# aicell-lab/bioengine-worker

Measured on AMD Instinct MI355X. Metric: cellpose_cyto3_512x512_imgs_per_sec, higher is better.
Workload: dtype bf16; 1 GPU; model=cellpose-cyto3 CPnet (nbase 2-32-64-128-256, style on, BN folded), global_batch=32, parallelism=dp1 (replica per GPU)

## Files before the change

bioengine_worker_amd/models/cpnet.py:

```python
from __future__ import annotations

import os
from dataclasses import dataclass

import torch
import torch.nn as nn
import torch.nn.functional as F

from ..ops import conv as convops
from ..ops import conv_pair as pairops
from ..ops import style as styleops


def _norm(c: int, kind: str) -> nn.Module:
    if kind == "batch":
        return nn.BatchNorm2d(c, eps=1e-5, momentum=0.05)
    if kind == "group":
        g = 8 if c % 8 == 0 else 1
        return nn.GroupNorm(g, c, eps=1e-5)
    raise ValueError(kind)


def batchconv(cin, cout, sz, norm="batch"):
    return nn.Sequential(_norm(cin, norm), nn.ReLU(inplace=True), nn.Conv2d(cin, cout, sz, padding=sz // 2))


def batchconv0(cin, cout, sz, norm="batch"):
    return nn.Sequential(_norm(cin, norm), nn.Conv2d(cin, cout, sz, padding=sz // 2))


class resdown(nn.Module):
    def __init__(self, cin, cout, sz, norm="batch"):
        super().__init__()
        self.conv = nn.Sequential()
        self.proj = batchconv0(cin, cout, 1, norm)
        for t in range(4):
            self.conv.add_module(f"conv_{t}", batchconv(cin if t == 0 else cout, cout, sz, norm))

    def forward(self, x):
        x = self.proj(x) + self.conv[1](self.conv[0](x))
        x = x + self.conv[3](self.conv[2](x))
        return x


class downsample(nn.Module):
    def __init__(self, nbase, sz, norm="batch"):
        super().__init__()
        self.down = nn.Sequential()
        self.maxpool = nn.MaxPool2d(2, 2)
        for n in range(len(nbase) - 1):
            self.down.add_module(f"res_down_{n}", resdown(nbase[n], nbase[n + 1], sz, norm))

    def forward(self, x):
        xd = []
        for n in range(len(self.down)):
            y = self.maxpool(xd[n - 1]) if n > 0 else x
            xd.append(self.down[n](y))
        return xd


class batchconvstyle(nn.Module):
    def __init__(self, cin, cout, style_channels, sz, norm="batch"):
        super().__init__()
        self.concatenation = False
        self.conv = batchconv(cin, cout, sz, norm)
        self.full = nn.Linear(style_channels, cout)

    def forward(self, style, x, y=None):
        if y is not None:
            x = x + y
        feat = self.full(style)
        return self.conv(x + feat.unsqueeze(-1).unsqueeze(-1))


class resup(nn.Module):
    def __init__(self, cin, cout, style_channels, sz, norm="batch"):
        super().__init__()
        self.conv = nn.Sequential()
        self.conv.add_module("conv_0", batchconv(cin, cout, sz, norm))
        self.conv.add_module("conv_1", batchconvstyle(cout, cout, style_channels, sz, norm))
        self.conv.add_module("conv_2", batchconvstyle(cout, cout, style_channels, sz, norm))
        self.conv.add_module("conv_3", batchconvstyle(cout, cout, style_channels, sz, norm))
        self.proj = batchconv0(cin, cout, 1, norm)

    def forward(self, x, y, style):
        x = self.proj(x) + self.conv[1](style, self.conv[0](x), y=y)
        x = x + self.conv[3](style, self.conv[2](style, x))
        return x


class make_style(nn.Module):
    def __init__(self):
        super().__init__()
        self.flatten = nn.Flatten()

    def forward(self, x0):
        style = F.avg_pool2d(x0, kernel_size=x0.shape[2:])
        style = self.flatten(style)
        return style / torch.sum(style ** 2, dim=1, keepdim=True) ** 0.5


class upsample(nn.Module):
    def __init__(self, nbase, sz, norm="batch"):
        super().__init__()
        self.upsampling = nn.Upsample(scale_factor=2, mode="nearest")
        self.up = nn.Sequential()
        for n in range(1, len(nbase)):
            self.up.add_module(f"res_up_{n - 1}", resup(nbase[n], nbase[n - 1], nbase[-1], sz, norm))

    def forward(self, style, xd):
        x = self.up[-1](xd[-1], xd[-1], style)
        for n in range(len(self.up) - 2, -1, -1):
            x = self.upsampling(x)
            x = self.up[n](x, xd[n], style)
        return x


class CPnet(nn.Module):

    def __init__(self, nbase=(2, 32, 64, 128, 256), nout=3, sz=3, diam_mean=30.0, norm="batch", style_on=True):
        super().__init__()
        nbase = list(nbase)
        self.nbase = nbase
        self.nout = nout
        self.sz = sz
        self.norm_kind = norm
        self.style_on = style_on
        self.downsample = downsample(nbase, sz, norm)
        nbaseup = nbase[1:] + [nbase[-1]]
        self.upsample = upsample(nbaseup, sz, norm)
        self.make_style = make_style()
        self.output = batchconv(nbaseup[0], nout, 1, norm)
        self.diam_mean = nn.Parameter(torch.ones(1) * diam_mean, requires_grad=False)
        self.diam_labels = nn.Parameter(torch.ones(1) * diam_mean, requires_grad=False)

    @property
    def nchan(self):
        return self.nbase[0]

    def forward(self, data):
        T0 = self.downsample(data)
        style = self.make_style(T0[-1])
        style0 = style
        if not self.style_on:
            style = style * 0
        T1 = self.upsample(style, T0)
        T1 = self.output(T1)
        return T1, style0, T0

    def randomize_(self, seed: int = 0) -> "CPnet":
        g = torch.Generator().manual_seed(seed)
        for m in self.modules():
            if isinstance(m, nn.Conv2d):
                fan_in = m.in_channels * m.kernel_size[0] * m.kernel_size[1]
                m.weight.data = torch.randn(m.weight.shape, generator=g) * (1.0 / fan_in) ** 0.5
                if m.bias is not None:
                    m.bias.data = torch.randn(m.bias.shape, generator=g) * 0.01
            elif isinstance(m, nn.Linear):
                m.weight.data = torch.randn(m.weight.shape, generator=g) * (1.0 / m.in_features) ** 0.5
                m.bias.data = torch.randn(m.bias.shape, generator=g) * 0.01
            elif isinstance(m, nn.BatchNorm2d):
                m.weight.data = 1.0 + 0.1 * torch.randn(m.weight.shape, generator=g)
                m.bias.data = 0.1 * torch.randn(m.bias.shape, generator=g)
                m.running_mean.data = 0.1 * torch.randn(m.running_mean.shape, generator=g)
                m.running_var.data = 1.0 + 0.1 * torch.rand(m.running_var.shape, generator=g)
            elif isinstance(m, nn.GroupNorm):
                m.weight.data = 1.0 + 0.1 * torch.randn(m.weight.shape, generator=g)
                m.bias.data = 0.1 * torch.randn(m.bias.shape, generator=g)
        return self



def _bn_fold(bn: nn.Module, device) -> tuple[torch.Tensor, torch.Tensor]:
    if isinstance(bn, nn.BatchNorm2d):
        s = bn.weight.detach().float() / torch.sqrt(bn.running_var.detach().float() + bn.eps)
        t = bn.bias.detach().float() - bn.running_mean.detach().float() * s
        return s.to(device).contiguous(), t.to(device).contiguous()
    raise TypeError("CPnetEngine folds eval-mode BatchNorm only; GroupNorm nets run the autograd path")


def _pad_vec(v: torch.Tensor, n: int, fill: float) -> torch.Tensor:
    if v.numel() == n:
        return v
    out = torch.full((n,), fill, dtype=v.dtype, device=v.device)
    out[: v.numel()] = v
    return out


class _FConv:

    def __init__(self, seq: nn.Sequential, relu: bool, device, cin_pad=None, cout_pad_to=None):
        bn, conv = seq[0], seq[-1]
        self.pc = convops.PackedConv.from_weight(conv.weight, conv.bias, cin_pad=cin_pad, cout_pad_to=cout_pad_to).to(device)
        if convops.pp128_build(self.pc) is not None and torch.device(device).type == "cuda":
            self.pc.frag()
        s, t = _bn_fold(bn, device)
        self.scale = _pad_vec(s, self.pc.cin_pad, 0.0)
        self.shift = _pad_vec(t, self.pc.cin_pad, 0.0)
        self.relu = relu

    def __call__(self, x, *, x2=None, shift=None, residual=None, inmode="none", out_nchw_f32=False, cout_valid=None,
                 residual_mode="full"):
        return convops.fused_conv2d(x, self.pc, x2=x2, scale=self.scale, shift=self.shift if shift is None else shift,
                                    relu=self.relu, residual=residual, inmode=inmode, out_nchw_f32=out_nchw_f32,
                                    cout_valid=cout_valid, residual_mode=residual_mode)


class _PPConv:

    def __init__(self, conv: nn.Conv2d, device, cfg: int | None = None):
        from ..ops import gemm_pp as ppops

        self.cout = conv.weight.shape[0]
        self.wp = ppops.pack_conv3(conv.weight).to(device)
        self.bias = None if conv.bias is None else conv.bias.detach().float().to(device).contiguous()
        self.cfg = cfg


def _igc(x, pk, **kw):
    if isinstance(pk, _PPConv):
        from ..ops import gemm_pp as ppops

        return ppops.conv3(x, pk.wp, pk.bias, cfg=pk.cfg, **kw)
    from ..ops import conv_igemm as igops

    return igops.conv3_igemm(x, pk, **kw)


@dataclass(frozen=True)
class CPnetEngineOptions:

    pair: bool = True
    pair_levels: tuple[int, ...] = (0, 1)
    igemm: str = "1"
    igemm_levels: tuple[int, ...] | None = (3,)
    head: bool = True
    pp_cfg: int | None = None

    @classmethod
    def from_env(cls) -> "CPnetEngineOptions":
        env = os.environ.get
        levels = lambda s: tuple(sorted({int(v) for v in s.split(",") if v.strip()}))
        ig_levels, cfg = env("BE_CPNET_IGEMM_LEVELS", "3"), env("BE_CPNET_PP_CFG")
        return cls(pair=env("BE_CPNET_PAIR", "1") != "0", pair_levels=levels(env("BE_CPNET_PAIR_LEVELS", "0,1")),
                   igemm=env("BE_CPNET_IGEMM", "1"), igemm_levels=levels(ig_levels) if ig_levels else None,
                   head=env("BE_CPNET_HEAD", "1") != "0", pp_cfg=None if cfg is None else int(cfg))


class CPnetEngine:

    def __init__(self, net: CPnet, device, options: CPnetEngineOptions | None = None):
        net = net.eval()
        self.options = opt = CPnetEngineOptions.from_env() if options is None else options
        self.device = torch.device(device)
        self.nout = net.nout
        self.nchan = net.nchan
        self.cin_pad = convops._round_up(net.nchan, 8)
        d = self.device
        self.down = []
        for n, blk in enumerate(net.downsample.down):
            cin_pad = self.cin_pad if n == 0 else None
            self.down.append(dict(
                proj=_FConv(blk.proj, False, d, cin_pad),
                c0=_FConv(blk.conv[0], True, d, cin_pad),
                c1=_FConv(blk.conv[1], True, d),
                c2=_FConv(blk.conv[2], True, d),
                c3=_FConv(blk.conv[3], True, d),
            ))
        self.up = []
        for blk in net.upsample.up:
            e = dict(proj=_FConv(blk.proj, False, d), c0=_FConv(blk.conv[0], True, d))
            for k in (1, 2, 3):
                bcs = blk.conv[k]
                e[f"c{k}"] = _FConv(bcs.conv, True, d)
                e[f"full{k}"] = (bcs.full.weight.detach().float().to(d), bcs.full.bias.detach().float().to(d))
            self.up.append(e)
        self.out = _FConv(net.output, True, d, cout_pad_to=16)
        self.style_on = net.style_on
        ws, bs, ss, ts = [], [], [], []
        self._feat_slices = []
        off = 0
        for i, e in enumerate(self.up):
            for k in (1, 2, 3):
                w, b = e[f"full{k}"]
                conv = e[f"c{k}"]
                ws.append(w); bs.append(b)
                ss.append(conv.scale[: w.shape[0]]); ts.append(conv.shift[: w.shape[0]])
                self._feat_slices.append((i, k, off, w.shape[0]))
                off += w.shape[0]
        self.style_w = torch.cat(ws, 0).contiguous()
        self.style_b = torch.cat(bs, 0).contiguous()
        self.style_s = torch.cat(ss, 0).contiguous()
        self.style_t = torch.cat(ts, 0).contiguous()
        self.pair = self._build_pairs(net) if opt.pair else {}
        self.ig_kind = opt.igemm
        self.ig = self._build_igemm(net) if self.ig_kind in ("1", "pp") else {}
        self.head = None
        if ("up", 0, 1) in self.pair and self.out.relu and self.nout <= 16 and opt.head:
            self.head = pairops.HeadSpec.build(self.out.scale, self.out.shift, net.output[-1].weight.to(d),
                                               None if net.output[-1].bias is None else net.output[-1].bias.to(d))

    def _build_pairs(self, net: CPnet) -> dict:
        nb = list(net.nbase)
        if len(nb) < 3 or nb[1] != 32 or nb[2] != 64 or self.cin_pad != 8 or net.sz != 3:
            return {}
        pairs = {}

        def spec(a: _FConv, b: _FConv, inmode="none", proj: _FConv | None = None, style_b=False, proj_rounded=False):
            bias = b.pc.bias if b.pc.bias is not None else torch.zeros(b.pc.cout, device=self.device)
            bias_p = None
            if proj is not None and proj_rounded:
                pb_ = proj.pc.bias if proj.pc.bias is not None else torch.zeros(proj.pc.cout, device=self.device)
                bias_p = pb_.float().contiguous()
            elif proj is not None and proj.pc.bias is not None:
                bias = bias + proj.pc.bias
            tb = None if style_b else pairops.fold_bias(b.shift, b.scale, a.pc.bias).contiguous()
            return pairops.PairSpec(pa=a.pc, pb=b.pc, sa=a.scale, ta=a.shift, sb=b.scale, tb=tb,
                                    bias=bias.float().contiguous(), inmode=inmode,
                                    pp=None if proj is None else proj.pc, sp=None if proj is None else proj.scale,
                                    tp=None if proj is None else proj.shift, bias_p=bias_p)

        d0, d1 = self.down[0], self.down[1]
        pairs[("down", 0, 0)] = spec(d0["c0"], d0["c1"], "none", proj=d0["proj"])
        pairs[("down", 0, 1)] = spec(d0["c2"], d0["c3"])
        pairs[("down", 1, 0)] = spec(d1["c0"], d1["c1"], "pool2", proj=d1["proj"], proj_rounded=True)
        pairs[("down", 1, 1)] = spec(d1["c2"], d1["c3"])
        nup = len(self.up)
        for i in (0, 1):
            if i >= nup - 1:
                continue
            e = self.up[i]
            pairs[("up", i, 0)] = spec(e["c0"], e["c1"], "up2", style_b=True)
            pairs[("up", i, 1)] = spec(e["c2"], e["c3"], style_b=True)
            for (ii, k, off, c) in self._feat_slices:
                if ii == i and k in (1, 3):
                    prev = e["c0"] if k == 1 else e["c2"]
                    if prev.pc.bias is not None:
                        self.style_t[off: off + c] += self.style_s[off: off + c] * prev.pc.bias[:c].to(self.device)
        pairs = {k: v for k, v in pairs.items() if k[1] in self.options.pair_levels}
        for key, sp in pairs.items():
            has_x2 = key[0] == "up" and key[2] == 0
            res = "none" if sp.pp is not None else ("up2" if has_x2 else "full")
            assert sp.supports(has_x2, res), key
            cfg = (sp.cin, sp.cm, sp.inmode, has_x2, sp.pp is not None, res)
            if cfg in pairops.FRAG_CONFIGS | pairops.PROJ_CONFIGS and torch.device(self.device).type == "cuda":
                sp.frag(sp.pa.wp.device)
                if cfg in pairops.PROJ_CONFIGS:
                    sp.frag_proj(sp.pa.wp.device)
        return pairs

    def _build_igemm(self, net: CPnet) -> dict:
        from ..ops import conv_igemm as igops
        from ..ops import gemm_pp as ppops

        ig = {}

        def add(key, conv: nn.Conv2d):
            cout, cin, kh, _ = conv.weight.shape
            if self.ig_kind == "pp":
                if kh == 3 and ppops.conv3_supported(cin, cout):
                    ig[key] = _PPConv(conv, self.device, self.options.pp_cfg)
            elif kh == 3 and cin % 16 == 0 and cout % 64 == 0:
                ig[key] = igops.IgemmConv.from_weight(conv.weight, conv.bias).to(self.device)

        nup = len(net.upsample.up)
        for n, blk in enumerate(net.downsample.down):
            if ("down", n, 0) in self.pair or n == 0:
                continue
            for k in (1, 2, 3):
                add(("down", n, k), blk.conv[k][-1])
        for i, blk in enumerate(net.upsample.up):
            if ("up", i, 0) in self.pair:
                continue
            if i == nup - 1:
                add(("up", i, 0), blk.conv[0][-1])
            for k in (1, 2, 3):
                add(("up", i, k), blk.conv[k].conv[-1])
        levels = {}
        for (kind, idx, k) in ig:
            levels.setdefault((kind, idx), set()).add(k)
        keep = self.options.igemm_levels
        full = {lv for lv, ks in levels.items() if ks >= {1, 2, 3} and (keep is None or lv[1] in keep)}
        return {key: v for key, v in ig.items() if (key[0], key[1]) in full}

    def _ig_level(self, kind: str, idx: int, x: torch.Tensor, H: int, W: int) -> bool:
        from ..ops import conv_igemm as igops

        pk = self.ig.get((kind, idx, 1))
        if pk is None or not x.is_cuda:
            return False
        if isinstance(pk, _PPConv):
            return True
        return igops.supported(x.shape[0], H, W, pk.cout, pk.bn)

    def _down_route(self, n: int, src: torch.Tensor) -> str:
        if n > 0 and ("down", n, 1) in self.ig and self._ig_level("down", n, src, src.shape[1] // 2, src.shape[2] // 2):
            return "ig"
        return "pair" if ("down", n, 0) in self.pair else "layer"

    def _down_pair(self, n: int, e: dict, src: torch.Tensor) -> torch.Tensor:
        P = self.pair
        if n == 0 or P[("down", n, 0)].pp is not None:
            x1 = pairops.conv_pair(src, P[("down", n, 0)])
        else:
            x1 = pairops.conv_pair(src, P[("down", n, 0)], res=e["proj"](src, inmode="pool2"), res_mode="full")
        return pairops.conv_pair(x1, P[("down", n, 1)], res=x1, res_mode="full")

    def _down_layer(self, n: int, e: dict, src: torch.Tensor) -> torch.Tensor:
        im = "pool2" if n > 0 else "none"
        if n > 0 and convops.pp128_takes_pool_proj(e["c0"].pc, e["proj"].pc, src):
            c0, pj = e["c0"], e["proj"]
            h, proj = convops.fused_conv2d_pool_proj(src, c0.pc, pj.pc, scale=c0.scale, shift=c0.shift, relu=c0.relu,
                                                     proj_scale=pj.scale, proj_shift=pj.shift)
        else:
            proj = e["proj"](src, inmode=im)
            h = e["c0"](src, inmode=im)
        x1 = e["c1"](h, residual=proj)
        h = e["c2"](x1)
        return e["c3"](h, residual=x1)

    def _down_ig(self, n: int, e: dict, src: torch.Tensor) -> tuple[torch.Tensor, torch.Tensor | None]:
        ig = self.ig
        c0, c1, c2, c3 = e["c0"], e["c1"], e["c2"], e["c3"]
        entry = convops.pp128_pooled_entry(c0.pc, src)
        if entry:
            pooled = convops.pool2_nhwc(src)
            proj = e["proj"](pooled)
            if entry == 2:
                ha = convops.fused_conv2d_c256(pooled, c0.pc, scale=c0.scale, shift=c0.shift, relu=True,
                                               post_scale=c1.scale, post_shift=c1.shift, post_relu=True)
            else:
                ha = convops.fused_conv2d(pooled, c0.pc, scale=c0.scale, shift=c0.shift, relu=True, nw=8,
                                          post_scale=c1.scale, post_shift=c1.shift, post_relu=True)
        else:
            proj = e["proj"](src, inmode="pool2")
            ha = convops.fused_conv2d(src, c0.pc, scale=c0.scale, shift=c0.shift, relu=True, inmode="pool2",
                                      post_scale=c1.scale, post_shift=c1.shift, post_relu=True)
        x1, x1a = _igc(ha, ig[("down", n, 1)], residual=proj, ascale=c2.scale, ashift=c2.shift)
        _, h2a = _igc(x1a, ig[("down", n, 2)], want_out=False, ascale=c3.scale, ashift=c3.shift)
        if n == len(self.down) - 1 and ("up", len(self.up) - 1, 0) in ig:
            nxt = self.up[-1]["c0"]
            return _igc(h2a, ig[("down", n, 3)], residual=x1, ascale=nxt.scale, ashift=nxt.shift)
        xd, _ = _igc(h2a, ig[("down", n, 3)], residual=x1)
        return xd, None

    def _up_route(self, i: int, xcur: torch.Tensor, top_act: torch.Tensor | None) -> str:
        same = i == len(self.up) - 1
        H, W = (xcur.shape[1], xcur.shape[2]) if same else (2 * xcur.shape[1], 2 * xcur.shape[2])
        if ("up", i, 1) in self.ig and (("up", i, 0) not in self.ig or top_act is not None) and \
                self._ig_level("up", i, xcur, H, W):
            return "ig"
        return "pair" if ("up", i, 0) in self.pair else "layer"

    def _up_pair(self, i: int, e: dict, xcur: torch.Tensor, y: torch.Tensor, shifts: dict) -> torch.Tensor:
        P = self.pair
        proj_lr = e["proj"](xcur)
        x1 = pairops.conv_pair(xcur, P[("up", i, 0)], tb=shifts[(i, 1)], x2=y, res=proj_lr, res_mode="up2")
        if i == 0 and self.head is not None:
            return pairops.conv_pair_head(x1, P[("up", 0, 1)], self.head, ta=shifts[(0, 2)], tb=shifts[(0, 3)], res=x1)
        return pairops.conv_pair(x1, P[("up", i, 1)], ta=shifts[(i, 2)], tb=shifts[(i, 3)], res=x1, res_mode="full")

    def _up_layer(self, i: int, e: dict, xcur: torch.Tensor, y: torch.Tensor, shifts: dict) -> torch.Tensor:
        im = "none" if i == len(self.up) - 1 else "up2"
        h0 = e["c0"](xcur, inmode=im, residual=y)
        if im == "up2" and xcur.is_cuda and convops.pp128_takes_res_up2(e["c1"].pc, h0):
            x1 = e["c1"](h0, shift=shifts[(i, 1)], residual=e["proj"](xcur), residual_mode="up2")
        else:
            x1 = e["c1"](h0, shift=shifts[(i, 1)], residual=e["proj"](xcur, inmode=im))
        h2 = e["c2"](x1, shift=shifts[(i, 2)])
        return e["c3"](h2, shift=shifts[(i, 3)], residual=x1)

    def _up_ig(self, i: int, e: dict, xcur: torch.Tensor, y: torch.Tensor, shifts: dict, xcur_act=None):
        ig = self.ig
        c1, c2, c3 = e["c1"], e["c2"], e["c3"]
        if ("up", i, 0) in ig:
            proj = e["proj"](xcur)
            _, h0a = _igc(xcur_act, ig[("up", i, 0)], residual=y, want_out=False, ascale=c1.scale,
                                       ashift=shifts[(i, 1)])
        else:
            proj = e["proj"](xcur, inmode="up2")
            h0a = convops.fused_conv2d(xcur, e["c0"].pc, scale=e["c0"].scale, shift=e["c0"].shift, relu=True,
                                       inmode="up2", residual=y, post_scale=c1.scale, post_shift=shifts[(i, 1)],
                                       post_relu=True)
        x1, x1a = _igc(h0a, ig[("up", i, 1)], residual=proj, ascale=c2.scale, ashift=shifts[(i, 2)])
        _, h2a = _igc(x1a, ig[("up", i, 2)], want_out=False, ascale=c3.scale, ashift=shifts[(i, 3)])
        out, _ = _igc(h2a, ig[("up", i, 3)], residual=x1)
        return out

    def _style_shifts(self, style: torch.Tensor) -> dict:
        st = style if self.style_on else torch.zeros_like(style)
        return self._split_shifts(styleops.style_shifts(st, self.style_w, self.style_b, self.style_s, self.style_t))

    def _split_shifts(self, shifts_all: torch.Tensor) -> dict:
        out = {}
        for (i, k, off, c) in self._feat_slices:
            out[(i, k)] = shifts_all[:, off: off + c]
        return out

    @torch.no_grad()
    def forward(self, x: torch.Tensor):
        xd = []
        nup = len(self.up)
        top_act = None
        for n, e in enumerate(self.down):
            src = x if n == 0 else xd[-1]
            route = self._down_route(n, src)
            if route == "ig":
                out, top_act = self._down_ig(n, e, src)
            else:
                out = self._down_pair(n, e, src) if route == "pair" else self._down_layer(n, e, src)
            xd.append(out)
        style, shifts_all = styleops.style_and_shifts(xd[-1], self.style_w, self.style_b, self.style_s, self.style_t,
                                                      self.style_on)
        shifts = self._split_shifts(shifts_all)
        xcur = xd[-1]
        for i in range(nup - 1, -1, -1):
            e = self.up[i]
            y = xd[i] if i < nup - 1 else xd[-1]
            route = self._up_route(i, xcur, top_act)
            if route == "ig":
                xcur = self._up_ig(i, e, xcur, y, shifts, top_act if i == nup - 1 else None)
            elif route == "pair":
                xcur = self._up_pair(i, e, xcur, y, shifts)
                if i == 0 and self.head is not None:
                    return xcur, style
            else:
                xcur = self._up_layer(i, e, xcur, y, shifts)
        return self.out(xcur, out_nchw_f32=True, cout_valid=self.nout), style

    __call__ = forward


def to_nhwc_input(x_nchw: torch.Tensor, cin_pad: int) -> torch.Tensor:
    N, C, H, W = x_nchw.shape
    out = torch.zeros(N, H, W, cin_pad, dtype=torch.bfloat16, device=x_nchw.device)
    out[..., :C] = x_nchw.permute(0, 2, 3, 1)
    return out
```

bioengine_worker_amd/ops/conv.py:

```python
from __future__ import annotations

import os

from dataclasses import dataclass

import torch
import torch.nn.functional as F

from . import _native

CK_1X1 = 64

INMODES = {"none": 0, "up2": 1, "pool2": 2}


def _round_up(v: int, m: int) -> int:
    return (v + m - 1) // m * m


@dataclass
class PackedConv:

    w: torch.Tensor
    bias: torch.Tensor | None
    ks: int
    cin: int
    cin_pad: int
    cout: int
    cout_pad: int
    ck: int
    tco: int
    kp: int
    wp: torch.Tensor | None = None
    wf: torch.Tensor | None = None
    wf_key: tuple | None = None

    @staticmethod
    def choose(cin_pad: int, cout: int, ks: int = 3) -> tuple[int, int]:
        ck = 8 if cin_pad % 32 else 32
        ck1 = int(os.environ.get("BE_CONV_CK1", CK_1X1))
        if ks == 1 and ck1 == 64 and cin_pad % 64 == 0:
            ck = 64
        if cout <= 16:
            tco = 16
        elif cout <= 32:
            tco = 32
        else:
            tco = 64
        return ck, tco

    @classmethod
    def from_weight(cls, weight: torch.Tensor, bias: torch.Tensor | None = None, cin_pad: int | None = None,
                    cout_pad_to: int | None = None, exact_cin: bool = False, ck16: bool = False) -> "PackedConv":
        cout, cin, ks, ks2 = weight.shape
        assert ks == ks2 and ks in (1, 3), "only 1x1 / 3x3 convs"
        cin_pad = cin_pad or _round_up(cin, 8)
        if cin_pad % 32 and cin_pad != 8 and not (exact_cin and cin_pad % 8 == 0):
            cin_pad = _round_up(cin_pad, 32)
        ck, tco = cls.choose(cin_pad, cout, ks)
        if ck16 and ks == 3 and ck == 8 and cin_pad % 16 == 0:
            ck = 16
        cout_k = max(cout, cout_pad_to or 0)
        cout_pad = _round_up(cout_k, tco)
        kp = ((ks * ks * ck + 31) // 32) * 32
        w = weight.detach().float()
        pc = cls(w=w, bias=None if bias is None else bias.detach().float(), ks=ks, cin=cin, cin_pad=cin_pad,
                 cout=cout, cout_pad=cout_pad, ck=ck, tco=tco, kp=kp)
        pc.wp = pc._pack(w)
        return pc

    def _pack(self, w: torch.Tensor) -> torch.Tensor:
        ks, ck = self.ks, self.ck
        nchunk = self.cin_pad // ck
        wz = torch.zeros(self.cout_pad, self.cin_pad, ks, ks, dtype=torch.float32, device=w.device)
        wz[: self.cout, : self.cin] = w
        t = wz.permute(0, 2, 3, 1).reshape(self.cout_pad, ks * ks, nchunk, ck)
        t = t.permute(0, 2, 1, 3).reshape(self.cout_pad, nchunk, ks * ks * ck)
        if self.kp > ks * ks * ck:
            t = F.pad(t, (0, self.kp - ks * ks * ck))
        return t.to(torch.bfloat16).contiguous()

    def to(self, device) -> "PackedConv":
        self.w = self.w.to(device)
        if self.bias is not None:
            self.bias = self.bias.to(device)
        built = self.wp is not None and self.frag_built() is not None
        if self.wp is not None:
            self.wp = self.wp.to(device)
        if built:
            self.wf = self.wf.to(device)
            self.wf_key = self._wp_key()
        return self

    def refresh(self, weight: torch.Tensor, bias: torch.Tensor | None = None) -> None:
        self.w = weight.detach().float()
        if bias is not None:
            self.bias = bias.detach().float()
        self.wp = self._pack(self.w)
        self.wf = self.wf_key = None

    def _wp_key(self) -> tuple:
        return (self.wp.data_ptr(), self.wp._version, str(self.wp.device))

    def frag(self) -> torch.Tensor:
        if self.frag_built() is None:
            pack = pack_frag_c256 if pp128_build(self) == "c256" else pack_frag if self.ks == 3 else pack_frag_1x1
            self.wf = pack(self.wp)
            self.wf_key = self._wp_key()
        return self.wf

    def frag_built(self) -> torch.Tensor | None:
        if self.wf is not None and self.wf_key == self._wp_key() and self.wf.device == self.wp.device:
            return self.wf
        return None


PP128_BUILDS = {(3, 128, 128): "c128", (3, 64, 128): "pool", (1, 64, 128): "proj", (3, 128, 256): "c256"}


def pp128_build(pc: PackedConv) -> str | None:
    if pc.cout_pad != pc.cout or (pc.ks == 3 and pc.ck != 32):
        return None
    return PP128_BUILDS.get((pc.ks, pc.cin_pad, pc.cout))


def frag_eligible(pc: PackedConv) -> bool:
    return pp128_build(pc) == "c128"


def frag_eligible_pool(pc: PackedConv) -> bool:
    return pp128_build(pc) == "pool"


def frag_eligible_proj(pc: PackedConv) -> bool:
    return pp128_build(pc) == "proj"


def frag_eligible_c256(pc: PackedConv) -> bool:
    return pp128_build(pc) == "c256"


def _pp128_takes(rule: str, x: torch.Tensor, *convs: tuple[PackedConv, str], pooled: bool = False,
                 frags: bool = True) -> bool:
    if not x.is_cuda:
        return False
    for pc, build in convs:
        if pp128_build(pc) != build or (frags and pc.frag_built() is None):
            return False
    N, H, W, _ = x.shape
    if pooled:
        if H % 2 or W % 2:
            return False
        H, W = H // 2, W // 2
    return bool(getattr(_native.hip(), "be_conv_pp128_takes_" + rule)(N, H, W))


def pp128_takes_prepool(pc: PackedConv, x: torch.Tensor) -> bool:
    return _pp128_takes("prepool", x, (pc, "c256"), pooled=True, frags=False)


def pp128_takes_c256(pc: PackedConv, x: torch.Tensor) -> bool:
    return _pp128_takes("c256", x, (pc, "c256"))


def pp128_pooled_entry(pc: PackedConv, x: torch.Tensor) -> int:
    if not pp128_takes_prepool(pc, x):
        return 0
    return 2 if _pp128_takes("c256", x, (pc, "c256"), pooled=True) else 1


def pp128_takes_pool(pc: PackedConv, x: torch.Tensor) -> bool:
    return _pp128_takes("pool", x, (pc, "pool"))


def pp128_takes_pool_proj(pc: PackedConv, pp: PackedConv, x: torch.Tensor) -> bool:
    return _pp128_takes("pool_proj", x, (pc, "pool"), (pp, "proj"))


def pp128_takes_res_up2(pc: PackedConv, x: torch.Tensor) -> bool:
    return not x.is_cuda or _pp128_takes("res_up2", x, (pc, "c128"))


def pack_frag_1x1(wp: torch.Tensor) -> torch.Tensor:
    cout, nchunk, kp = wp.shape
    assert cout % 16 == 0 and nchunk * kp == 64, "fragment packing: a 1x1 conv of 64 input channels, whole channel tiles"
    nct = cout // 16
    t = wp.reshape(nct, 16, 2, 4, 8)
    return t.permute(2, 0, 3, 1, 4).contiguous().reshape(2, nct, 64, 8)


def pack_frag(wp: torch.Tensor) -> torch.Tensor:
    cout, nchunk, kp = wp.shape
    assert cout % 16 == 0 and kp == 288, "fragment packing: 3x3 taps of 32-channel chunks, whole channel tiles"
    nct = cout // 16
    t = wp.reshape(nct, 16, nchunk, 9, 4, 8)
    return t.permute(2, 3, 0, 4, 1, 5).contiguous().reshape(nchunk, 9, nct, 64, 8)


def pack_frag_c256(wp: torch.Tensor) -> torch.Tensor:
    cout, nchunk, kp = wp.shape
    assert cout == 256 and nchunk == 4 and kp == 288, "fragment packing: a 3x3 conv of 128 -> 256 channels"
    return torch.stack([pack_frag(wp[:128]), pack_frag(wp[128:])]).contiguous()


def unpack_frag(wf: torch.Tensor) -> torch.Tensor:
    nchunk, _, nct = wf.shape[:3]
    t = wf.reshape(nchunk, 9, nct, 4, 16, 8)
    return t.permute(2, 4, 0, 1, 3, 5).contiguous().reshape(nct * 16, nchunk, 288)


register = _native.register_hip_signatures


def _act_ref(x, x2, scale, shift, relu, inmode):
    xt = x.permute(0, 3, 1, 2)
    if inmode == "up2":
        xt = F.interpolate(xt, scale_factor=2, mode="nearest")
    elif inmode == "pool2":
        xt = F.max_pool2d(xt, 2, 2)
    if x2 is not None:
        xt = xt + x2.permute(0, 3, 1, 2).float()
    C = xt.shape[1]
    if scale is not None:
        xt = xt * (scale.view(-1, C, 1, 1) if scale.dim() == 2 else scale.view(1, C, 1, 1))
    if shift is not None:
        sh = shift.view(-1, C, 1, 1) if shift.dim() == 2 else shift.view(1, C, 1, 1)
        xt = xt + sh
    if relu:
        xt = torch.relu(xt)
    return xt


def fused_conv2d_ref(x, pc: PackedConv, x2=None, scale=None, shift=None, relu=False, residual=None,
                     inmode="none", out_nchw_f32=False, cout_valid=None, act_dtype=torch.bfloat16, post_relu=False,
                     no_bias=False):
    a = _act_ref(x.float(), x2, scale, shift, relu, inmode)
    if act_dtype is not None:
        a = a.to(act_dtype).float()
    w = pc.w.to(a.device)
    if w.shape[1] < a.shape[1]:
        w = F.pad(w, (0, 0, 0, 0, 0, a.shape[1] - w.shape[1]))
    wq = w.to(torch.bfloat16).float() if act_dtype is not None else w
    y = F.conv2d(a, wq, None, padding=pc.ks // 2)
    if pc.bias is not None and not no_bias:
        y = y + pc.bias.to(y.device).view(1, -1, 1, 1)
    if out_nchw_f32:
        cv = cout_valid or pc.cout
        y = y[:, :cv].contiguous()
        return torch.relu(y) if post_relu else y
    y = y.permute(0, 2, 3, 1)
    if residual is not None:
        y = y + residual.float()
    if post_relu:
        y = torch.relu(y)
    return y.to(x.dtype).contiguous()


NW_POLICY: dict = {}
DEFAULT_NW = None


def choose_nw(pc: PackedConv, H: int, W: int, inmode: str = "none", has_x2: bool = False) -> int:
    key = (pc.ks, pc.cin_pad, pc.cout, inmode)
    if key in NW_POLICY:
        return NW_POLICY[key]
    if DEFAULT_NW is not None:
        return DEFAULT_NW
    if pc.tco <= 32:
        return 8
    if has_x2:
        return 4
    if inmode == "pool2" and pc.ks == 3 and H * W <= 28 * 28:
        return 8
    return 4


def _affine_stride(t: torch.Tensor | None, N: int, C: int) -> int:
    if t is None:
        return 0
    assert t.dtype == torch.float32
    if t.dim() == 2:
        assert t.shape == (N, C) and t.stride(1) == 1, "per-image affine must be [N, C] with unit column stride"
        ns = t.stride(0) if N > 1 else C
        assert ns % 4 == 0 and t.data_ptr() % 16 == 0, "per-image affine rows must be 16-byte aligned"
        return ns
    assert t.is_contiguous() and t.numel() == C
    return 0


def out_hw(x: torch.Tensor, inmode: str) -> tuple[int, int]:
    _, Hs, Ws, _ = x.shape
    if inmode == "up2":
        return 2 * Hs, 2 * Ws
    if inmode == "pool2":
        return Hs // 2, Ws // 2
    return Hs, Ws


def fused_conv2d(x: torch.Tensor, pc: PackedConv, *, x2=None, scale=None, shift=None, relu=False, residual=None,
                 inmode: str = "none", out_nchw_f32: bool = False, cout_valid: int | None = None,
                 nw: int | None = None, post_relu: bool = False, out: torch.Tensor | None = None,
                 no_bias: bool = False, post_scale=None, post_shift=None, residual_mode: str = "full") -> torch.Tensor:
    N, Hs, Ws, Cin = x.shape
    H, W = out_hw(x, inmode)
    assert residual_mode in ("full", "up2")
    up2 = residual is not None and residual_mode == "up2"
    if up2:
        assert H % 2 == 0 and W % 2 == 0 and residual.shape == (N, H // 2, W // 2, pc.cout)
    if not x.is_cuda:
        if up2:
            residual = residual.repeat_interleave(2, dim=1).repeat_interleave(2, dim=2)
        y = fused_conv2d_ref(x, pc, x2, scale, shift, relu, residual, inmode, out_nchw_f32, cout_valid,
                             act_dtype=torch.bfloat16 if x.dtype == torch.bfloat16 else None,
                             post_relu=post_relu and post_scale is None and post_shift is None, no_bias=no_bias)
        if post_scale is not None or post_shift is not None:
            yf = y.to(torch.bfloat16).float()
            if post_scale is not None:
                yf = yf * post_scale.to(yf.device)
            if post_shift is not None:
                ps = post_shift.to(yf.device)
                yf = yf + (ps[:, None, None, :] if ps.dim() == 2 else ps)
            if post_relu:
                yf = torch.relu(yf)
            y = yf.to(y.dtype)
        if out is not None:
            out.copy_(y)
            return out
        return y
    assert x.dtype == torch.bfloat16 and x.is_contiguous(), "fused_conv2d expects contiguous NHWC bf16"
    assert Cin == pc.cin_pad, f"input channels {Cin} != packed cin {pc.cin_pad}"
    if pc.wp.device != x.device:
        pc.to(x.device)
    cout_valid = cout_valid or pc.cout
    if out_nchw_f32:
        assert out is None
        out = torch.empty(N, cout_valid, H, W, device=x.device, dtype=torch.float32)
        cout_store = pc.cout_pad
    else:
        assert pc.cout % 4 == 0
        if out is None:
            out = torch.empty(N, H, W, pc.cout, device=x.device, dtype=torch.bfloat16)
        else:
            assert out.shape == (N, H, W, pc.cout) and out.dtype == torch.bfloat16 and out.is_contiguous()
        cout_store = pc.cout
    if x2 is not None:
        assert x2.shape == (N, H, W, Cin) and x2.dtype == torch.bfloat16 and x2.is_contiguous()
    if residual is not None:
        assert residual.shape == ((N, H // 2, W // 2, pc.cout) if up2 else (N, H, W, pc.cout))
        assert residual.dtype == torch.bfloat16 and residual.is_contiguous()
    pscale_ns = _affine_stride(scale, N, Cin)
    pshift_ns = _affine_stride(shift, N, Cin)
    qshift_ns = _affine_stride(post_shift, N, pc.cout)
    if post_scale is not None:
        assert post_scale.dtype == torch.float32 and post_scale.is_contiguous() and post_scale.numel() == pc.cout
    build = pp128_build(pc)
    wf = pc.frag_built() if build == "c128" or (build == "pool" and inmode == "pool2") else None
    args = (
        _native.ptr(x), _native.ptr(x2), _native.ptr(scale), _native.ptr(shift), pshift_ns, pscale_ns,
        int(bool(relu)) | (2 if post_relu else 0),
        _native.ptr(pc.wp), _native.ptr(None if no_bias else pc.bias), _native.ptr(residual), _native.ptr(out),
        N, H, W, Hs, Ws, Cin, cout_store, cout_valid, pc.ks, pc.ck, pc.tco, INMODES[inmode], int(out_nchw_f32),
        int(nw or choose_nw(pc, H, W, inmode, x2 is not None)), _native.ptr(post_scale), _native.ptr(post_shift),
        qshift_ns, _native.ptr(wf),
    )
    if up2:
        _native.call("be_conv2d_nhwc_frag_res", *args, 1, _native.stream(x.device))
    else:
        _native.call("be_conv2d_nhwc_frag", *args, _native.stream(x.device))
    return out


def fused_conv2d_pool_proj(x: torch.Tensor, pc: PackedConv, pp: PackedConv, *, scale, shift, relu: bool, proj_scale,
                           proj_shift) -> tuple[torch.Tensor, torch.Tensor]:
    N, Hs, Ws, Cin = x.shape
    assert x.is_cuda and x.dtype == torch.bfloat16 and x.is_contiguous() and Cin == 64 == pc.cin_pad == pp.cin_pad
    assert frag_eligible_pool(pc) and frag_eligible_proj(pp)
    wf, wpf = pc.frag_built(), pp.frag_built()
    assert wf is not None and wpf is not None, "fragment-order weights are packed when the engine is built"
    assert proj_scale.dtype == proj_shift.dtype == torch.float32 and proj_scale.numel() == proj_shift.numel() == 64
    assert proj_scale.is_contiguous() and proj_shift.is_contiguous()
    H, W = Hs // 2, Ws // 2
    out = torch.empty(N, H, W, 128, device=x.device, dtype=torch.bfloat16)
    out2 = torch.empty(N, H, W, 128, device=x.device, dtype=torch.bfloat16)
    _native.call("be_conv_pp128_pool_proj", _native.ptr(x), _native.ptr(scale), _native.ptr(shift),
                 _affine_stride(shift, N, Cin), _affine_stride(scale, N, Cin), int(bool(relu)), _native.ptr(wf),
                 _native.ptr(pc.bias), _native.ptr(out), _native.ptr(proj_scale), _native.ptr(proj_shift), _native.ptr(wpf),
                 _native.ptr(pp.bias), _native.ptr(out2), N, Hs, Ws, _native.stream(x.device))
    return out, out2


def pool2_nhwc_ref(x: torch.Tensor) -> torch.Tensor:
    def mx(p, q):
        return torch.where((p > q) | ((p == q) & ~torch.signbit(p)), p, q)

    return mx(mx(x[:, 0::2, 0::2], x[:, 0::2, 1::2]), mx(x[:, 1::2, 0::2], x[:, 1::2, 1::2])).contiguous()


def pool2_nhwc(x: torch.Tensor, out: torch.Tensor | None = None) -> torch.Tensor:
    N, Hs, Ws, C = x.shape
    assert Hs % 2 == 0 and Ws % 2 == 0, "pool2_nhwc needs an even source size"
    if not x.is_cuda:
        y = pool2_nhwc_ref(x)
        if out is not None:
            out.copy_(y)
            return out
        return y
    assert x.dtype == torch.bfloat16 and x.is_contiguous() and C % 8 == 0, "pool2_nhwc expects contiguous NHWC bf16"
    if out is None:
        out = torch.empty(N, Hs // 2, Ws // 2, C, device=x.device, dtype=torch.bfloat16)
    else:
        assert out.shape == (N, Hs // 2, Ws // 2, C) and out.dtype == torch.bfloat16 and out.is_contiguous()
    _native.call("be_pool2_nhwc", _native.ptr(x), _native.ptr(out), N, Hs, Ws, C, _native.stream(x.device))
    return out


def fused_conv2d_c256(x: torch.Tensor, pc: PackedConv, *, scale, shift, relu: bool, post_scale, post_shift,
                      post_relu: bool) -> torch.Tensor:
    N, H, W, Cin = x.shape
    assert x.is_cuda and x.dtype == torch.bfloat16 and x.is_contiguous() and Cin == 128 == pc.cin_pad
    assert frag_eligible_c256(pc)
    wf = pc.frag_built()
    assert wf is not None, "fragment-order weights are packed when the engine is built"
    for q in (post_scale, post_shift):
        assert q is not None and q.dtype == torch.float32 and q.is_contiguous() and q.dim() == 1 and q.numel() == 256
    out = torch.empty(N, H, W, 256, device=x.device, dtype=torch.bfloat16)
    _native.call("be_conv_pp128_c256", _native.ptr(x), _native.ptr(scale), _native.ptr(shift),
                 _affine_stride(shift, N, Cin), _affine_stride(scale, N, Cin), int(bool(relu)) | (2 if post_relu else 0),
                 _native.ptr(wf), _native.ptr(pc.bias), _native.ptr(out), _native.ptr(post_scale), _native.ptr(post_shift),
                 N, H, W, _native.stream(x.device))
    return out


def depth_to_space2(y: torch.Tensor, c: int) -> torch.Tensor:
    N, H, W, _ = y.shape
    return y.view(N, H, W, 2, 2, c).permute(0, 1, 3, 2, 4, 5).reshape(N, 2 * H, 2 * W, c)


def fused_conv2d_concat(xa: torch.Tensor, xb: torch.Tensor, pc: PackedConv, *, post_relu: bool = False,
                        nw: int | None = None, xb_d2s: bool = False) -> torch.Tensor:
    N, H, W, Ca = xa.shape
    Cb = xb.shape[-1] // 4 if xb_d2s else xb.shape[-1]
    if xb_d2s:
        assert xb.shape[:3] == (N, H // 2, W // 2) and H % 2 == 0 and W % 2 == 0
    else:
        assert xb.shape[:3] == (N, H, W)
    assert pc.ks == 3 and pc.cin_pad == Ca + Cb
    if not xa.is_cuda:
        xbf = depth_to_space2(xb, Cb) if xb_d2s else xb
        return fused_conv2d(torch.cat([xa, xbf], -1), pc, post_relu=post_relu)
    assert xa.dtype == xb.dtype == torch.bfloat16 and xa.is_contiguous() and xb.is_contiguous()
    assert Ca % 8 == 0 and Cb % 8 == 0 and pc.cout % 4 == 0
    if pc.wp.device != xa.device:
        pc.to(xa.device)
    out = torch.empty(N, H, W, pc.cout, device=xa.device, dtype=torch.bfloat16)
    _native.call("be_conv2d_concat", _native.ptr(xa), _native.ptr(xb), _native.ptr(pc.wp), _native.ptr(pc.bias),
                 _native.ptr(out), N, H, W, Ca, Cb, pc.cout, pc.ck, pc.tco, int(bool(post_relu)),
                 int(nw or choose_nw(pc, H, W)), int(bool(xb_d2s)), _native.stream(xa.device))
    return out
```

csrc/kernels/conv_pair.hip:

```cpp
#include <cstdlib>

#include "common.h"

namespace {

struct PairArgs {
  const bf16_t* x;
  const bf16_t* x2;
  const float* sa; const float* ta; int ta_ns;
  const float* sb; const float* tb; int tb_ns;
  const float* sp; const float* tp;
  const bf16_t* wa;
  const bf16_t* wb;
  const bf16_t* wp;
  const float* bias;
  const bf16_t* waf; const bf16_t* wbf;
  const bf16_t* wpf; const float* biasp;
  const bf16_t* res;
  bf16_t* out;
  const float* sh; const float* th;
  const bf16_t* wh;
  const float* bh;
  float* hout;
  int nh;
  int N, H, W, Hs, Ws, Cin;
  int tiles_x, tiles_y;
  unsigned long long* stamps;
};

namespace g32 {
constexpr int TW = 32, TH = 16, NW = 8;
#include "conv_pair_onegroup.inc"
}
using namespace g32;

unsigned long long* g_pair_stamps = nullptr;
int g_pair_stamps_cap = 0;

static int g_pair_var = (be_env_int("BE_PAIR_LATE_EPI", 1) ? 1 : 0) | (be_env_int("BE_PAIR_ROLL", 1) ? 2 : 0) |
                        (be_env_int("BE_PAIR_EARLY_AFF", 1) ? 4 : 0) | (be_env_int("BE_PAIR_EPIA", 0) ? 8 : 0) |
                        (be_env_int("BE_PAIR_SEPS", 0) ? 16 : 0) | (be_env_int("BE_PAIR_TOPEPI", 0) ? 32 : 0);

template <int CK, int CM, int INMODE, bool X2, bool PROJ, int RES, int NCA, bool HEAD, bool STAMP, int VAR>
int launch_pair_l(PairArgs a, int g, hipStream_t s) {
  using C = PC<CK, CM, INMODE, X2, PROJ, RES, NCA>;
  constexpr bool seps = (VAR & 16) != 0 && C::RESW && !HEAD;
  constexpr size_t lds = C::LDS + (seps ? (size_t)C::R_OUT * sizeof(bf16_t) : 0);
  static_assert(lds <= 160 * 1024, "LDS budget (separate output staging)");
  static bool attr_set[BE_MAX_DEV] = {};
  if (!attr_set[be_cur_dev()]) {
    hipFuncSetAttribute(
        reinterpret_cast<const void*>(&conv_pair_kernel<CK, CM, INMODE, X2, PROJ, RES, NCA, HEAD, STAMP, VAR>),
        hipFuncAttributeMaxDynamicSharedMemorySize, (int)lds);
    attr_set[be_cur_dev()] = true;
  }
  hipLaunchKernelGGL((conv_pair_kernel<CK, CM, INMODE, X2, PROJ, RES, NCA, HEAD, STAMP, VAR>), dim3(g), dim3(NT), lds, s,
                     a);
  return BE_CHECK_LAUNCH();
}

template <int CK, int CM, int INMODE, bool X2, bool PROJ, int RES, int NCA, bool HEAD = false, bool STAMP = false>
int launch_pair_k(PairArgs a, int g, hipStream_t s) {
  if constexpr (CM == 32 && CK == 32 && !HEAD) {
    if (g_pair_var & 16) {
      if constexpr (NCA == 1)
        if (g_pair_var & 32) return launch_pair_l<CK, CM, INMODE, X2, PROJ, RES, NCA, HEAD, STAMP, 48>(a, g, s);
      return launch_pair_l<CK, CM, INMODE, X2, PROJ, RES, NCA, HEAD, STAMP, 16>(a, g, s);
    }
  }
  if constexpr (CM == 32 && NCA == 1) {
    if (g_pair_var & 32) return launch_pair_l<CK, CM, INMODE, X2, PROJ, RES, NCA, HEAD, STAMP, 32>(a, g, s);
  }
  if constexpr (CM == 64 && RES != 0) {
    switch (g_pair_var & 15) {
      case 1: return launch_pair_l<CK, CM, INMODE, X2, PROJ, RES, NCA, HEAD, STAMP, 1>(a, g, s);
      case 2: return launch_pair_l<CK, CM, INMODE, X2, PROJ, RES, NCA, HEAD, STAMP, 2>(a, g, s);
      case 3: return launch_pair_l<CK, CM, INMODE, X2, PROJ, RES, NCA, HEAD, STAMP, 3>(a, g, s);
      case 5: return launch_pair_l<CK, CM, INMODE, X2, PROJ, RES, NCA, HEAD, STAMP, 5>(a, g, s);
      case 7: return launch_pair_l<CK, CM, INMODE, X2, PROJ, RES, NCA, HEAD, STAMP, 7>(a, g, s);
      case 15: return launch_pair_l<CK, CM, INMODE, X2, PROJ, RES, NCA, HEAD, STAMP, 15>(a, g, s);
      default: break;
    }
  }
  return launch_pair_l<CK, CM, INMODE, X2, PROJ, RES, NCA, HEAD, STAMP, 0>(a, g, s);
}

template <int CK, int CM, int INMODE, bool X2, bool PROJ, int RES, int NCA, bool HEAD = false>
int launch_pair(PairArgs a, int grid_cap, hipStream_t s) {
  a.tiles_x = (a.W + TW - 1) / TW;
  a.tiles_y = (a.H + TH - 1) / TH;
  const int tiles = a.N * a.tiles_x * a.tiles_y;
  int g = grid_cap > 0 ? grid_cap : 256;
  if (g > tiles) g = tiles;
  if (g < 1) return 0;
  a.stamps = nullptr;
  if constexpr (!HEAD && !PROJ && CK == 32) {
    if (g_pair_stamps != nullptr) {
      if (g > g_pair_stamps_cap) return -30;
      a.stamps = g_pair_stamps;
      return launch_pair_k<CK, CM, INMODE, X2, PROJ, RES, NCA, HEAD, true>(a, g, s);
    }
  }
  return launch_pair_k<CK, CM, INMODE, X2, PROJ, RES, NCA, HEAD, false>(a, g, s);
}

#ifndef PP_VAR
#define PP_VAR 1
#endif
#ifndef PP_GW
#define PP_GW 4
#endif
namespace ppk {
constexpr int GW = PP_GW, GT = GW * 64;
constexpr int NTP = 2 * GT;
constexpr int RPW = TH / GW;
constexpr int IN_B = IPIX * 64;
constexpr int H_B = RPIX * 64;
constexpr int OUTW_B = RPW * TW * 64;
constexpr int RB = IN_B;
constexpr int WSTR = 9 * 32 + 16;
constexpr int W_B = 32 * WSTR * 2;
constexpr int APT = 40 / GW, BPT = 32 / GW;
constexpr int TLAST0 = GW * (APT - 1);
constexpr int HU = IPIX * 4;
constexpr int HUPT = (HU + GT - 1) / GT;
static_assert(H_B <= RB && GW * OUTW_B <= RB, "ping-pong region overlays");
static_assert(APT * GW >= RPT && (APT - 1) * GW <= 2 * RH && BPT * GW * 16 == TH * TW, "tile maps");
static_assert(GW == 4 || GW == 8, "group size");
}

struct PPHalo {
  u32x4 h[ppk::HUPT];
  float4 aff[4];
};

__device__ __forceinline__ int pp_in_off(int pi, int c) {
  const int y = pi / IW, x = pi - y * IW;
  return pi * 64 + ((c ^ ((((x >> 2) ^ y) & 1) << 1)) << 4);
}

template <int INMODE, int CIN, bool INT = false>
__device__ __forceinline__ void pp_issue_halo(const PairArgs& a, TileXY t, int ch, int gt, PPHalo& hr) {
  const int c = ch * 32 + (gt & 3) * 8;
  hr.aff[0] = *reinterpret_cast<const float4*>(a.sa + c);
  hr.aff[1] = *reinterpret_cast<const float4*>(a.sa + c + 4);
  const float* tr = a.ta + (size_t)t.n * a.ta_ns + c;
  hr.aff[2] = *reinterpret_cast<const float4*>(tr);
  hr.aff[3] = *reinterpret_cast<const float4*>(tr + 4);
#pragma unroll
  for (int i = 0; i < ppk::HUPT; ++i) {
    const int pi = min(gt + i * ppk::GT, ppk::HU - 1) >> 2;
    const int y = pi / IW, x = pi - y * IW;
    const int gy = INT ? t.ty0 - 2 + y : min(max(t.ty0 - 2 + y, 0), a.H - 1);
    const int gx = INT ? t.tx0 - 2 + x : min(max(t.tx0 - 2 + x, 0), a.W - 1);
    if constexpr (INMODE == 0)
      hr.h[i] = *reinterpret_cast<const u32x4*>(a.x + (((size_t)t.n * a.Hs + gy) * a.Ws + gx) * CIN + c);
    else
      hr.h[i] = *reinterpret_cast<const u32x4*>(a.x + (((size_t)t.n * a.Hs + (gy >> 1)) * a.Ws + (gx >> 1)) * CIN + c);
  }
}

__device__ __forceinline__ bool pp_interior(const PairArgs& a, TileXY t) {
  return t.ty0 >= 2 && t.ty0 + TH + 2 <= a.H && t.tx0 >= 2 && t.tx0 + TW + 2 <= a.W;
}

template <bool INT>
__device__ __forceinline__ void pp_commit(const PairArgs& a, TileXY t, int gt, const PPHalo& hr, unsigned char* rin) {
  float sc[8], sh[8];
  unpack_aff(hr.aff, sc, sh);
  const int c = gt & 3;
#pragma unroll
  for (int i = 0; i < ppk::HUPT; ++i) {
    const int u = gt + i * ppk::GT;
    if (u >= ppk::HU) continue;
    const int pi = u >> 2;
    const int y = pi / IW, x = pi - y * IW;
    const int gy = t.ty0 - 2 + y, gx = t.tx0 - 2 + x;
    u32x4 pk = (u32x4){0u, 0u, 0u, 0u};
    if (INT || (gy >= 0 && gy < a.H && gx >= 0 && gx < a.W)) {
#pragma unroll
      for (int j = 0; j < 4; ++j)
        pk[j] = relu_bf16x2(pack2bf(fmaf(lo_bf(hr.h[i][j]), sc[2 * j], sh[2 * j]),
                                    fmaf(hi_bf(hr.h[i][j]), sc[2 * j + 1], sh[2 * j + 1])));
    }
    *reinterpret_cast<u32x4*>(rin + pi * 64 + ((c ^ ((((x >> 2) ^ y) & 1) << 1)) << 4)) = pk;
  }
}

__device__ __forceinline__ void pp_mma_a(f32x4 (&acc)[2][ppk::APT], const unsigned char* rin, const bf16_t* wa, int gw,
                                         int lrow, int kq) {
  const int par = (gw >> 1) & 1;
  const int b0 = ((gw >> 1) * IW + (gw & 1) * 16 + lrow) * 64;
  int A0[3][2];
#pragma unroll
  for (int dx = 0; dx < 3; ++dx)
#pragma unroll
    for (int pr = 0; pr < 2; ++pr)
      A0[dx][pr] = b0 + dx * 64 + ((kq ^ (((((lrow + dx) >> 2) ^ par ^ pr) & 1) << 1)) << 4);
  int L[3][2];
  const int tl = gw + ppk::TLAST0;
  if (tl < 2 * RH) {
    const int ryl = tl >> 1, rxl = (tl & 1) * 16 + lrow;
#pragma unroll
    for (int dx = 0; dx < 3; ++dx)
#pragma unroll
      for (int pr = 0; pr < 2; ++pr)
        L[dx][pr] = (ryl * IW + rxl + dx) * 64 + ((kq ^ (((((lrow + dx) >> 2) ^ ryl ^ pr) & 1) << 1)) << 4);
  } else {
    int ry9 = (tl - 2 * RH) * 8 + (lrow >> 1), rx9 = 32 + (lrow & 1);
    if (ry9 >= RH) { ry9 = 0; rx9 = 0; }
#pragma unroll
    for (int dx = 0; dx < 3; ++dx)
#pragma unroll
      for (int pr = 0; pr < 2; ++pr)
        L[dx][pr] = (ry9 * IW + rx9 + dx) * 64 + ((kq ^ ((((ry9 & 1) ^ pr) & 1) << 1)) << 4);
  }
  auto frags = [&](int ks, bf16x8 (&af)[2], bf16x8 (&bf)[ppk::APT]) {
    const int dy = ks / 3, dx = ks % 3;
#pragma unroll
    for (int ct = 0; ct < 2; ++ct)
      af[ct] = *reinterpret_cast<const bf16x8*>(wa + (ct * 16 + lrow) * ppk::WSTR + ks * 32 + kq * 8);
#pragma unroll
    for (int j = 0; j < ppk::APT - 1; ++j)
      bf[j] = *reinterpret_cast<const bf16x8*>(rin + A0[dx][dy & 1] + j * (ppk::GW / 2) * IW * 64 + dy * IW * 64);
    bf[ppk::APT - 1] = *reinterpret_cast<const bf16x8*>(rin + L[dx][dy & 1] + dy * IW * 64);
  };
  bf16x8 af[2], afn[2], bf[ppk::APT];
  frags(0, af, bf);
#pragma unroll
  for (int ks = 0; ks < 9; ++ks) {
    const bool more = ks + 1 < 9;
    const int kn = more ? ks + 1 : ks, dy = kn / 3, dx = kn % 3;
#pragma unroll
    for (int j = 0; j < ppk::APT; ++j) {
#pragma unroll
      for (int ct = 0; ct < 2; ++ct) {
        acc[ct][j] = __builtin_amdgcn_mfma_f32_16x16x32_bf16(af[ct], bf[j], acc[ct][j], 0, 0, 0);
        if (j == 0 && more)
          afn[ct] = *reinterpret_cast<const bf16x8*>(wa + (ct * 16 + lrow) * ppk::WSTR + kn * 32 + kq * 8);
      }
      if (more) {
        if (j < ppk::APT - 1)
          bf[j] = *reinterpret_cast<const bf16x8*>(rin + A0[dx][dy & 1] + j * (ppk::GW / 2) * IW * 64 + dy * IW * 64);
        else
          bf[j] = *reinterpret_cast<const bf16x8*>(rin + L[dx][dy & 1] + dy * IW * 64);
      }
      __builtin_amdgcn_sched_barrier(0);
    }
    if (more) {
      af[0] = afn[0];
      af[1] = afn[1];
    }
  }
}

struct PPSkip {
  u32x2 xv[ppk::APT][2];
};

__device__ __forceinline__ bool pp_last(int gw, int lrow, int& ry, int& rx) {
  const int tl = gw + ppk::TLAST0;
  if (tl < 2 * RH) {
    ry = tl >> 1;
    rx = (tl & 1) * 16 + lrow;
    return true;
  }
  ry = (tl - 2 * RH) * 8 + (lrow >> 1);
  rx = 32 + (lrow & 1);
  return ry < RH;
}

__device__ __forceinline__ void pp_issue_skip(const PairArgs& a, TileXY t, int gw, int lrow, int kq, PPSkip& sk) {
#pragma unroll
  for (int j = 0; j < ppk::APT; ++j) {
    int ry, rx;
    if (j < ppk::APT - 1) {
      ry = (gw >> 1) + (ppk::GW / 2) * j;
      rx = (gw & 1) * 16 + lrow;
    } else {
      pp_last(gw, lrow, ry, rx);
    }
    const int gy = min(max(t.ty0 - 1 + ry, 0), a.H - 1), gx = min(max(t.tx0 - 1 + rx, 0), a.W - 1);
    const bf16_t* xp = a.x2 + (((size_t)t.n * a.H + gy) * a.W + gx) * 32 + kq * 4;
#pragma unroll
    for (int ct = 0; ct < 2; ++ct) sk.xv[j][ct] = *reinterpret_cast<const u32x2*>(xp + ct * 16);
  }
}

template <bool X2, bool INT>
__device__ __forceinline__ void pp_epi_a(const PairArgs& a, TileXY t, const f32x4 (&acc)[2][ppk::APT],
                                         unsigned char* rh, const float4 (&s)[2], const float4 (&sh)[2],
                                         const PPSkip& sk, int gw, int lrow, int kq) {
#pragma unroll
  for (int ct = 0; ct < 2; ++ct) {
    const int hc = ((2 * ct) | (kq >> 1));
    const int hw = (((gw >> 1) * RW + (gw & 1) * 16 + lrow) * 64) + ((hc ^ ((lrow >> 1) & 3)) << 4) + (kq & 1) * 8;
#pragma unroll
    for (int j = 0; j < ppk::APT; ++j) {
      int ry, rx, off;
      if (j < ppk::APT - 1) {
        ry = (gw >> 1) + (ppk::GW / 2) * j;
        rx = (gw & 1) * 16 + lrow;
        off = hw + j * (ppk::GW / 2) * RW * 64;
      } else {
        if (!pp_last(gw, lrow, ry, rx)) continue;
        off = (ry * RW + rx) * 64 + ((hc ^ ((rx >> 1) & 3)) << 4) + (kq & 1) * 8;
      }
      const int gy = t.ty0 - 1 + ry, gx = t.tx0 - 1 + rx;
      float v0 = acc[ct][j][0], v1 = acc[ct][j][1], v2 = acc[ct][j][2], v3 = acc[ct][j][3];
      if constexpr (X2) {
        u32x2 xv = sk.xv[j][ct];
        asm volatile("" : "+v"(xv));
        v0 += lo_bf(xv[0]); v1 += hi_bf(xv[0]); v2 += lo_bf(xv[1]); v3 += hi_bf(xv[1]);
      }
      u32x2 st = (u32x2){0u, 0u};
      if (INT || (gy >= 0 && gy < a.H && gx >= 0 && gx < a.W)) {
        st[0] = relu_bf16x2(pack2bf(fmaf(v0, s[ct].x, sh[ct].x), fmaf(v1, s[ct].y, sh[ct].y)));
        st[1] = relu_bf16x2(pack2bf(fmaf(v2, s[ct].z, sh[ct].z), fmaf(v3, s[ct].w, sh[ct].w)));
      }
      *reinterpret_cast<u32x2*>(rh + off) = st;
    }
  }
}

__device__ __forceinline__ void pp_mma_b(f32x4 (&acc)[2][ppk::BPT], const unsigned char* rh, const bf16_t* wb, int gw,
                                         int lrow, int kq) {
  int B0[3];
#pragma unroll
  for (int dx = 0; dx < 3; ++dx) B0[dx] = ((ppk::RPW * gw) * RW + lrow + dx) * 64 + ((kq ^ (((lrow + dx) >> 1) & 3)) << 4);
  auto frags = [&](int ks, bf16x8 (&af)[2], bf16x8 (&bf)[ppk::BPT]) {
    const int dy = ks / 3, dx = ks % 3;
#pragma unroll
    for (int ct = 0; ct < 2; ++ct)
      af[ct] = *reinterpret_cast<const bf16x8*>(wb + (ct * 16 + lrow) * ppk::WSTR + ks * 32 + kq * 8);
#pragma unroll
    for (int pt = 0; pt < ppk::BPT; ++pt)
      bf[pt] = *reinterpret_cast<const bf16x8*>(rh + B0[dx] + ((pt >> 1) + dy) * RW * 64 + (pt & 1) * 16 * 64);
  };
  bf16x8 af[2], afn[2], bf[ppk::BPT];
  frags(0, af, bf);
#pragma unroll
  for (int ks = 0; ks < 9; ++ks) {
    const bool more = ks + 1 < 9;
    const int kn = more ? ks + 1 : ks, dy = kn / 3, dx = kn % 3;
#pragma unroll
    for (int pt = 0; pt < ppk::BPT; ++pt) {
#pragma unroll
      for (int ct = 0; ct < 2; ++ct) {
        acc[ct][pt] = __builtin_amdgcn_mfma_f32_16x16x32_bf16(af[ct], bf[pt], acc[ct][pt], 0, 0, 0);
        if (pt == 0 && more)
          afn[ct] = *reinterpret_cast<const bf16x8*>(wb + (ct * 16 + lrow) * ppk::WSTR + kn * 32 + kq * 8);
      }
      if (more) bf[pt] = *reinterpret_cast<const bf16x8*>(rh + B0[dx] + ((pt >> 1) + dy) * RW * 64 + (pt & 1) * 16 * 64);
      __builtin_amdgcn_sched_barrier(0);
    }
    if (more) {
      af[0] = afn[0];
      af[1] = afn[1];
    }
  }
}

struct PPRes {
  u32x2 rv[ppk::BPT][2];
  float4 bias[2];
};

template <int RES>
__device__ __forceinline__ void pp_issue_res(const PairArgs& a, TileXY t, int gw, int lrow, int kq, PPRes& r) {
#pragma unroll
  for (int pt = 0; pt < ppk::BPT; ++pt) {
    if constexpr (RES == 0) {
      r.rv[pt][0] = r.rv[pt][1] = (u32x2){0u, 0u};
      continue;
    }
    const int py = min(t.ty0 + ppk::RPW * gw + (pt >> 1), a.H - 1), px = min(t.tx0 + (pt & 1) * 16 + lrow, a.W - 1);
    const bf16_t* rp = RES == 1 ? a.res + (((size_t)t.n * a.H + py) * a.W + px) * 32 + kq * 4
                                : a.res + (((size_t)t.n * (a.H >> 1) + (py >> 1)) * (a.W >> 1) + (px >> 1)) * 32 + kq * 4;
#pragma unroll
    for (int ct = 0; ct < 2; ++ct) r.rv[pt][ct] = *reinterpret_cast<const u32x2*>(rp + ct * 16);
  }
#pragma unroll
  for (int ct = 0; ct < 2; ++ct) r.bias[ct] = *reinterpret_cast<const float4*>(a.bias + ct * 16 + kq * 4);
}

template <int RES>
__device__ __forceinline__ void pp_epi_b(const PairArgs& a, TileXY t, const f32x4 (&acc)[2][ppk::BPT], const PPRes& r,
                                         unsigned char* ws, int gw, int lrow, int kq, bool act) {
  const __amdgpu_buffer_rsrc_t rs = __builtin_amdgcn_make_buffer_rsrc(
      a.out + (size_t)t.n * a.H * a.W * 32, (short)0, a.H * a.W * 64, 0x00020000);
  if constexpr (PP_VAR & 16) {
#pragma unroll
    for (int pt = 0; pt < ppk::BPT; ++pt) {
      const int py = t.ty0 + ppk::RPW * gw + (pt >> 1), px = t.tx0 + (pt & 1) * 16 + lrow;
      const bool ok = act && py < a.H && px < a.W;
#pragma unroll
      for (int ct = 0; ct < 2; ++ct) {
        u32x2 rv = r.rv[pt][ct];
        asm volatile("" : "+v"(rv));
        u32x2 st;
        st[0] = pack2bf(acc[ct][pt][0] + r.bias[ct].x + lo_bf(rv[0]), acc[ct][pt][1] + r.bias[ct].y + hi_bf(rv[0]));
        st[1] = pack2bf(acc[ct][pt][2] + r.bias[ct].z + lo_bf(rv[1]), acc[ct][pt][3] + r.bias[ct].w + hi_bf(rv[1]));
        const int off = ok ? ((py * a.W + px) * 32 + ct * 16 + kq * 4) * 2 : 0x7ffffff0;
        __builtin_amdgcn_raw_buffer_store_b64(st, rs, off, 0, 0);
      }
    }
    return;
  }
#pragma unroll
  for (int ct = 0; ct < 2; ++ct) {
    const int ow = lrow * 64 + ((((2 * ct) | (kq >> 1)) ^ ((lrow >> 1) & 3)) << 4) + (kq & 1) * 8;
#pragma unroll
    for (int pt = 0; pt < ppk::BPT; ++pt) {
      u32x2 rv = r.rv[pt][ct];
      if constexpr (RES != 0) asm volatile("" : "+v"(rv));
      u32x2 st;
      st[0] = pack2bf(acc[ct][pt][0] + r.bias[ct].x + lo_bf(rv[0]), acc[ct][pt][1] + r.bias[ct].y + hi_bf(rv[0]));
      st[1] = pack2bf(acc[ct][pt][2] + r.bias[ct].z + lo_bf(rv[1]), acc[ct][pt][3] + r.bias[ct].w + hi_bf(rv[1]));
      *reinterpret_cast<u32x2*>(ws + ow + ((pt >> 1) * 32 + (pt & 1) * 16) * 64) = st;
    }
  }
  __builtin_amdgcn_fence(__ATOMIC_RELEASE, "wavefront");
  __builtin_amdgcn_wave_barrier();
  __builtin_amdgcn_fence(__ATOMIC_ACQUIRE, "wavefront");
  const int lane = lrow + 16 * kq;
  const int rd = (lane >> 2) * 64 + (((lane & 3) ^ ((lane >> 3) & 3)) << 4);
  const int py0 = t.ty0 + ppk::RPW * gw, px0 = t.tx0 + (lane >> 2);
#pragma unroll
  for (int it = 0; it < 2 * ppk::RPW; ++it) {
    const int py = py0 + (it >> 1), px = px0 + (it & 1) * 16;
    const u32x4 v = *reinterpret_cast<const u32x4*>(ws + rd + it * 1024);
    const int off = (act && py < a.H && px < a.W) ? ((py * a.W + px) * 32 + (lane & 3) * 8) * 2 : 0x7ffffff0;
    __builtin_amdgcn_raw_buffer_store_b128(v, rs, off, 0, 0);
    __builtin_amdgcn_sched_barrier(0);
  }
}

__device__ __forceinline__ void pp_epi_head(const PairArgs& a, TileXY t, const f32x4 (&acc)[2][ppk::BPT], const PPRes& r,
                                            const HeadRegs& hr, int gw, int lrow, int kq, bool act) {
  const f32x4 zero = {0.f, 0.f, 0.f, 0.f};
  const __amdgpu_buffer_rsrc_t rs = __builtin_amdgcn_make_buffer_rsrc(
      a.hout + (size_t)t.n * a.nh * a.H * a.W, (short)0, a.nh * a.H * a.W * 4, 0x00020000);
#pragma unroll
  for (int pt = 0; pt < ppk::BPT; ++pt) {
    u32x4 bw;
#pragma unroll
    for (int ct = 0; ct < 2; ++ct) {
      u32x2 rv = r.rv[pt][ct];
      asm volatile("" : "+v"(rv));
      const float4 bias = r.bias[ct];
      const uint32_t o0 = pack2bf(acc[ct][pt][0] + bias.x + lo_bf(rv[0]), acc[ct][pt][1] + bias.y + hi_bf(rv[0]));
      const uint32_t o1 = pack2bf(acc[ct][pt][2] + bias.z + lo_bf(rv[1]), acc[ct][pt][3] + bias.w + hi_bf(rv[1]));
      bw[2 * ct] = relu_bf16x2(pack2bf(fmaf(lo_bf(o0), hr.s[ct].x, hr.t[ct].x), fmaf(hi_bf(o0), hr.s[ct].y, hr.t[ct].y)));
      bw[2 * ct + 1] = relu_bf16x2(pack2bf(fmaf(lo_bf(o1), hr.s[ct].z, hr.t[ct].z), fmaf(hi_bf(o1), hr.s[ct].w, hr.t[ct].w)));
    }
    const f32x4 y = __builtin_amdgcn_mfma_f32_16x16x32_bf16(hr.w, *reinterpret_cast<const bf16x8*>(&bw), zero, 0, 0, 0);
    const int py = t.ty0 + ppk::RPW * gw + (pt >> 1), px = t.tx0 + (pt & 1) * 16 + lrow;
    const bool ok = act && py < a.H && px < a.W;
    const float bb[4] = {hr.b.x, hr.b.y, hr.b.z, hr.b.w};
#pragma unroll
    for (int i = 0; i < 4; ++i) {
      const int co = kq * 4 + i;
      const int off = (ok && co < a.nh) ? ((co * a.H + py) * a.W + px) * 4 : 0x7ffffff0;
      __builtin_amdgcn_raw_buffer_store_b32(__float_as_uint(y[i] + bb[i]), rs, off, 0, 0);
    }
  }
}

namespace pps {
constexpr int PST = 24;
constexpr int PSP = 8;
constexpr int KPA = 96, WSTRA = KPA + 16;
constexpr int WSTRP = 48;
constexpr int IN_B = IPIX * PST * 2;
constexpr int P_B = TH * TW * PSP * 2;
constexpr int R_B = ppk::H_B > IN_B ? ppk::H_B : IN_B;
constexpr int RB = R_B + P_B;
constexpr int WA_B = 32 * WSTRA * 2, WB_B = 32 * ppk::WSTR * 2, WP_B = 32 * WSTRP * 2;
constexpr int LDS = 2 * RB + WA_B + WB_B + WP_B;
constexpr int HUPT = (IPIX + ppk::GT - 1) / ppk::GT;
static_assert(LDS <= 128 * 1024 && ppk::GW * ppk::OUTW_B <= R_B, "stem ping-pong LDS budget");
}

struct PPHalo8 {
  u32x4 h[pps::HUPT];
  float4 aff[4], paff[4];
};

template <bool INT = false>
__device__ __forceinline__ void pp8_issue_halo(const PairArgs& a, TileXY t, int gt, PPHalo8& hr) {
  hr.aff[0] = *reinterpret_cast<const float4*>(a.sa);
  hr.aff[1] = *reinterpret_cast<const float4*>(a.sa + 4);
  const float* tr = a.ta + (size_t)t.n * a.ta_ns;
  hr.aff[2] = *reinterpret_cast<const float4*>(tr);
  hr.aff[3] = *reinterpret_cast<const float4*>(tr + 4);
  hr.paff[0] = *reinterpret_cast<const float4*>(a.sp);
  hr.paff[1] = *reinterpret_cast<const float4*>(a.sp + 4);
  hr.paff[2] = *reinterpret_cast<const float4*>(a.tp);
  hr.paff[3] = *reinterpret_cast<const float4*>(a.tp + 4);
#pragma unroll
  for (int i = 0; i < pps::HUPT; ++i) {
    const int pi = min(gt + i * ppk::GT, IPIX - 1);
    const int y = pi / IW, x = pi - y * IW;
    const int gy = INT ? t.ty0 - 2 + y : min(max(t.ty0 - 2 + y, 0), a.H - 1);
    const int gx = INT ? t.tx0 - 2 + x : min(max(t.tx0 - 2 + x, 0), a.W - 1);
    hr.h[i] = *reinterpret_cast<const u32x4*>(a.x + (((size_t)t.n * a.Hs + gy) * a.Ws + gx) * 8);
  }
}

template <bool INT>
__device__ __forceinline__ void pp8_commit(const PairArgs& a, TileXY t, int gt, const PPHalo8& hr, unsigned char* rin,
                                           unsigned char* preg) {
  float sc[8], sh[8], ps[8], pt[8];
  unpack_aff(hr.aff, sc, sh);
  unpack_aff(hr.paff, ps, pt);
#pragma unroll
  for (int i = 0; i < pps::HUPT; ++i) {
    const int pi = gt + i * ppk::GT;
    if (pi >= IPIX) continue;
    const int iy = pi / IW, ix = pi - iy * IW;
    const int gy = t.ty0 - 2 + iy, gx = t.tx0 - 2 + ix;
    const bool in = INT || (gy >= 0 && gy < a.H && gx >= 0 && gx < a.W);
    float v[8];
#pragma unroll
    for (int j = 0; j < 4; ++j) { v[2 * j] = lo_bf(hr.h[i][j]); v[2 * j + 1] = hi_bf(hr.h[i][j]); }
    u32x4 pk = (u32x4){0u, 0u, 0u, 0u};
    if (in) {
#pragma unroll
      for (int j = 0; j < 4; ++j)
        pk[j] = relu_bf16x2(pack2bf(fmaf(v[2 * j], sc[2 * j], sh[2 * j]), fmaf(v[2 * j + 1], sc[2 * j + 1], sh[2 * j + 1])));
    }
    *reinterpret_cast<u32x4*>(rin + pi * pps::PST * 2) = pk;
    if (iy >= 2 && iy < TH + 2 && ix >= 2 && ix < TW + 2) {
      u32x4 pp = (u32x4){0u, 0u, 0u, 0u};
      if (in) {
#pragma unroll
        for (int j = 0; j < 4; ++j)
          pp[j] = pack2bf(fmaf(v[2 * j], ps[2 * j], pt[2 * j]), fmaf(v[2 * j + 1], ps[2 * j + 1], pt[2 * j + 1]));
      }
      *reinterpret_cast<u32x4*>(preg + ((iy - 2) * TW + (ix - 2)) * pps::PSP * 2) = pp;
    }
  }
}

__device__ __forceinline__ void pp8_mma_a(f32x4 (&acc)[2][ppk::APT], const unsigned char* rin, const bf16_t* wa, int gw,
                                          int lrow, int kq) {
  int toff[3];
#pragma unroll
  for (int ks = 0; ks < 3; ++ks) {
    int tap = ks * 4 + kq;
    if (tap >= 9) tap = 0;
    toff[ks] = ((tap / 3) * IW + tap % 3) * pps::PST * 2;
  }
  const int b0 = ((gw >> 1) * IW + (gw & 1) * 16 + lrow) * pps::PST * 2;
  int ryl, rxl;
  if (!pp_last(gw, lrow, ryl, rxl)) { ryl = 0; rxl = 0; }
  const int bl = (ryl * IW + rxl) * pps::PST * 2;
#pragma unroll
  for (int ks = 0; ks < 3; ++ks) {
    bf16x8 af[2], bf[ppk::APT];
#pragma unroll
    for (int ct = 0; ct < 2; ++ct)
      af[ct] = *reinterpret_cast<const bf16x8*>(wa + (ct * 16 + lrow) * pps::WSTRA + ks * 32 + kq * 8);
#pragma unroll
    for (int j = 0; j < ppk::APT - 1; ++j)
      bf[j] = *reinterpret_cast<const bf16x8*>(rin + b0 + toff[ks] + j * (ppk::GW / 2) * IW * pps::PST * 2);
    bf[ppk::APT - 1] = *reinterpret_cast<const bf16x8*>(rin + bl + toff[ks]);
#pragma unroll
    for (int ct = 0; ct < 2; ++ct)
#pragma unroll
      for (int j = 0; j < ppk::APT; ++j)
        acc[ct][j] = __builtin_amdgcn_mfma_f32_16x16x32_bf16(af[ct], bf[j], acc[ct][j], 0, 0, 0);
  }
}

__device__ __forceinline__ void pp8_mma_p(f32x4 (&acc)[2][ppk::BPT], const unsigned char* preg, const bf16_t* wp, int gw,
                                          int lrow, int kq) {
  bf16x8 af[2], bf[ppk::BPT];
#pragma unroll
  for (int ct = 0; ct < 2; ++ct) af[ct] = *reinterpret_cast<const bf16x8*>(wp + (ct * 16 + lrow) * pps::WSTRP + kq * 8);
#pragma unroll
  for (int pt = 0; pt < ppk::BPT; ++pt) {
    const int oy = ppk::RPW * gw + (pt >> 1), ox = (pt & 1) * 16 + lrow;
    bf[pt] = *reinterpret_cast<const bf16x8*>(preg + (oy * TW + ox) * pps::PSP * 2);
  }
#pragma unroll
  for (int ct = 0; ct < 2; ++ct)
#pragma unroll
    for (int pt = 0; pt < ppk::BPT; ++pt)
      acc[ct][pt] = __builtin_amdgcn_mfma_f32_16x16x32_bf16(af[ct], bf[pt], acc[ct][pt], 0, 0, 0);
}

template <bool STEM> struct PPHaloOf { using T = PPHalo; };
template <> struct PPHaloOf<true> { using T = PPHalo8; };

template <int NCA, int INMODE, bool X2, int RES, bool HEAD, bool STEM = false, bool STAMP = false>
__global__ __launch_bounds__(ppk::NTP, ppk::GW == 4 ? 2 : 4) void conv_pair_pp_kernel(PairArgs a) {
  static_assert(!STEM || (NCA == 1 && INMODE == 0 && !X2 && RES == 0 && !HEAD), "stem configuration");
  constexpr int CIN = 32 * NCA;
  constexpr int RB = STEM ? pps::RB : ppk::RB;
  unsigned long long ph_work[7] = {0, 0, 0, 0, 0, 0, 0}, ph_wait[7] = {0, 0, 0, 0, 0, 0, 0};
  unsigned long long tstamp = STAMP ? __builtin_amdgcn_s_memtime() : 0;
  auto pre = [&](int i) {
    if constexpr (STAMP) {
      const unsigned long long tn = __builtin_amdgcn_s_memtime();
      ph_work[i] += tn - tstamp;
      tstamp = tn;
    }
  };
  auto post = [&](int i) {
    if constexpr (STAMP) {
      const unsigned long long tn = __builtin_amdgcn_s_memtime();
      ph_wait[i] += tn - tstamp;
      tstamp = tn;
    }
  };
  constexpr int NST = HEAD ? 4 * ppk::BPT : ((PP_VAR & 16) ? 2 * ppk::BPT : 2 * ppk::RPW);
  extern __shared__ __attribute__((aligned(16))) unsigned char smem[];
  const int tid0 = threadIdx.x;
  const int total = a.N * a.tiles_x * a.tiles_y;
  const int t0 = (int)(((long long)blockIdx.x * total) / gridDim.x);
  const int t1 = (int)(((long long)(blockIdx.x + 1) * total) / gridDim.x);
  if (t0 >= t1) return;
  bf16_t* wl = reinterpret_cast<bf16_t*>(smem + 2 * RB);
  const bf16_t* wb = wl + (STEM ? 32 * pps::WSTRA : NCA * 32 * ppk::WSTR);
  const bf16_t* wp = wb + 32 * ppk::WSTR;
  if constexpr (STEM) {
    for (int u = tid0; u < 32 * (12 + 36 + 4); u += ppk::NTP) {
      const int r = u / 52, q = u % 52;
      const bf16_t* src;
      bf16_t* dst;
      if (q < 12) { src = a.wa + (size_t)r * 96 + q * 8; dst = wl + r * pps::WSTRA + q * 8; }
      else if (q < 48) { src = a.wb + (size_t)r * 288 + (q - 12) * 8; dst = const_cast<bf16_t*>(wb) + r * ppk::WSTR + (q - 12) * 8; }
      else { src = a.wp + (size_t)r * 32 + (q - 48) * 8; dst = const_cast<bf16_t*>(wp) + r * pps::WSTRP + (q - 48) * 8; }
      *reinterpret_cast<u32x4*>(dst) = *reinterpret_cast<const u32x4*>(src);
    }
  } else {
    for (int u = tid0; u < (NCA + 1) * 32 * 36; u += ppk::NTP) {
      const int pnl = u / (32 * 36), q = u % (32 * 36), r = q / 36, k8 = q % 36;
      const bf16_t* src = pnl < NCA ? a.wa + ((size_t)r * NCA + pnl) * 288 + k8 * 8 : a.wb + (size_t)r * 288 + k8 * 8;
      *reinterpret_cast<u32x4*>(wl + pnl * 32 * ppk::WSTR + r * ppk::WSTR + k8 * 8) = *reinterpret_cast<const u32x4*>(src);
    }
  }
  const int grp = __builtin_amdgcn_readfirstlane(tid0 / ppk::GT);
  const int gt0 = tid0 & (ppk::GT - 1);
  unsigned char* reg = smem + grp * RB;
  HeadRegs hr;
  if constexpr (HEAD) load_head(a, tid0 & 15, (tid0 & 63) >> 4, hr);
  typename PPHaloOf<STEM>::T halo;
  auto issue0 = [&](TileXY nx, int gtv) {
    if constexpr (STEM) {
      if (pp_interior(a, nx)) pp8_issue_halo<true>(a, nx, gtv, halo);
      else pp8_issue_halo<false>(a, nx, gtv, halo);
    } else {
      if (pp_interior(a, nx)) pp_issue_halo<INMODE, CIN, true>(a, nx, 0, gtv, halo);
      else pp_issue_halo<INMODE, CIN>(a, nx, 0, gtv, halo);
    }
  };
  if constexpr (STEM) pp8_issue_halo<false>(a, tile_xy(a, min(t0 + grp, t1 - 1)), gt0, halo);
  else pp_issue_halo<INMODE, CIN>(a, tile_xy(a, min(t0 + grp, t1 - 1)), 0, gt0, halo);
  __builtin_amdgcn_s_waitcnt((0x7 << 4) | (0xf << 8));
  __syncthreads();
  if (grp == 1) __builtin_amdgcn_s_barrier();
  const int iters = (t1 - t0 + 1) >> 1;
  for (int k = 0; k < iters; ++k) {
    int gt = gt0;
    asm volatile("" : "+v"(gt));
    const int gw = __builtin_amdgcn_readfirstlane(gt >> 6), lane = gt & 63, lrow = lane & 15, kq = lane >> 4;
    const int t = t0 + 2 * k + grp;
    const bool act = t < t1;
    const TileXY cur = tile_xy(a, act ? t : t1 - 1);
    const bool inner = pp_interior(a, cur);
    f32x4 acc_a[2][ppk::APT];
    float4 sb[2], tb[2];
    PPSkip sk;
#pragma unroll
    for (int c = 0; c < NCA; ++c) {
      constexpr int NW = (PP_VAR & 2) ? 0 : NST;
      if (c == 0) __builtin_amdgcn_s_waitcnt((NW & 0xf) | (0x7 << 4) | (0xf << 8) | ((NW >> 4) << 14));
      int gc = gt0;
      asm volatile("" : "+v"(gc));
      if constexpr (STEM) {
        if (inner) pp8_commit<true>(a, cur, gc, halo, reg, reg + pps::R_B);
        else pp8_commit<false>(a, cur, gc, halo, reg, reg + pps::R_B);
      } else {
        if (inner) pp_commit<true>(a, cur, gc, halo, reg);
        else pp_commit<false>(a, cur, gc, halo, reg);
      }
      pre(2 * c);
      __syncthreads();
      post(2 * c);
      if constexpr (!STEM) {
        if (c + 1 < NCA) {
          if (inner) pp_issue_halo<INMODE, CIN, true>(a, cur, c + 1, gt, halo);
          else pp_issue_halo<INMODE, CIN>(a, cur, c + 1, gt, halo);
        }
      }
      if (c == NCA - 1) {
#pragma unroll
        for (int ct = 0; ct < 2; ++ct) {
          sb[ct] = *reinterpret_cast<const float4*>(a.sb + ct * 16 + kq * 4);
          tb[ct] = *reinterpret_cast<const float4*>(a.tb + (size_t)cur.n * a.tb_ns + ct * 16 + kq * 4);
        }
        if constexpr (X2) pp_issue_skip(a, cur, gw, lrow, kq, sk);
      }
      if (c == 0) {
#pragma unroll
        for (int i = 0; i < 2; ++i)
#pragma unroll
          for (int j = 0; j < ppk::APT; ++j) acc_a[i][j] = (f32x4){0.f, 0.f, 0.f, 0.f};
      }
      if constexpr (!(PP_VAR & 4)) __builtin_amdgcn_s_setprio(1);
      if constexpr (STEM) pp8_mma_a(acc_a, reg, wl, gw, lrow, kq);
      else pp_mma_a(acc_a, reg, wl + c * 32 * ppk::WSTR, gw, lrow, kq);
      if constexpr (!(PP_VAR & 4)) __builtin_amdgcn_s_setprio(0);
      pre(2 * c + 1);
      __syncthreads();
      post(2 * c + 1);
    }
    int g3 = gt0;
    asm volatile("" : "+v"(g3));
    if (inner) pp_epi_a<X2, true>(a, cur, acc_a, reg, sb, tb, sk, gw, g3 & 15, (g3 & 63) >> 4);
    else pp_epi_a<X2, false>(a, cur, acc_a, reg, sb, tb, sk, gw, g3 & 15, (g3 & 63) >> 4);
    PPRes res;
    if constexpr (PP_VAR & 1) pp_issue_res<RES>(a, cur, gw, g3 & 15, (g3 & 63) >> 4, res);
    if constexpr (PP_VAR & 8) issue0(tile_xy(a, min(t + 2, t1 - 1)), g3);
    pre(2 * NCA);
    __syncthreads();
    post(2 * NCA);
    int g4 = gt0;
    asm volatile("" : "+v"(g4));
    const int lrow4 = g4 & 15, kq4 = (g4 & 63) >> 4;
    f32x4 acc_b[2][ppk::BPT];
    if constexpr (!(PP_VAR & 1)) pp_issue_res<RES>(a, cur, gw, lrow4, kq4, res);
#pragma unroll
    for (int i = 0; i < 2; ++i)
#pragma unroll
      for (int j = 0; j < ppk::BPT; ++j) acc_b[i][j] = (f32x4){0.f, 0.f, 0.f, 0.f};
    if constexpr (!(PP_VAR & 4)) __builtin_amdgcn_s_setprio(1);
    pp_mma_b(acc_b, reg, wb, gw, lrow4, kq4);
    if constexpr (STEM) pp8_mma_p(acc_b, reg + pps::R_B, wp, gw, lrow4, kq4);
    if constexpr (!(PP_VAR & 4)) __builtin_amdgcn_s_setprio(0);
    pre(2 * NCA + 1);
    __syncthreads();
    post(2 * NCA + 1);
    int g5 = gt0;
    asm volatile("" : "+v"(g5));
    const int lrow5 = g5 & 15, kq5 = (g5 & 63) >> 4;
    auto next_halo = [&]() { issue0(tile_xy(a, min(t + 2, t1 - 1)), g5); };
    if constexpr (!(PP_VAR & 10)) next_halo();
    __builtin_amdgcn_sched_barrier(0);
    if constexpr (HEAD) pp_epi_head(a, cur, acc_b, res, hr, gw, lrow5, kq5, act);
    else pp_epi_b<RES>(a, cur, acc_b, res, reg + gw * ppk::OUTW_B, gw, lrow5, kq5, act);
    if constexpr (PP_VAR & 2) next_halo();
    pre(2 * NCA + 2);
    __syncthreads();
    post(2 * NCA + 2);
  }
  if (grp == 0) __builtin_amdgcn_s_barrier();
  if constexpr (STAMP) {
    if ((tid0 & (ppk::GT - 1)) < 16) {
      const int k = tid0 & 15;
      unsigned long long v = 0;
#pragma unroll
      for (int i = 0; i < 7; ++i) {
        if (k == i) v = ph_work[i];
        if (k == 8 + i) v = ph_wait[i];
      }
      if (k == 15) v = (unsigned long long)iters;
      a.stamps[((size_t)blockIdx.x * 2 + grp) * 16 + k] = v;
    }
  }
}

unsigned long long* g_pp_stamps = nullptr;
int g_pp_stamps_cap = 0;

template <int NCA, int INMODE, bool X2, int RES, bool HEAD, bool STEM = false>
int launch_pair_pp(PairArgs a, int grid_cap, hipStream_t s) {
  constexpr int lds = STEM ? pps::LDS : 2 * ppk::RB + (NCA + 1) * ppk::W_B;
  static_assert(lds <= 160 * 1024, "ping-pong LDS budget");
  a.tiles_x = (a.W + TW - 1) / TW;
  a.tiles_y = (a.H + TH - 1) / TH;
  const int tiles = a.N * a.tiles_x * a.tiles_y;
  int g = grid_cap > 0 ? grid_cap : 256;
  if (g > tiles) g = tiles;
  if (g < 1) return 0;
  a.stamps = nullptr;
  static bool attr_set[BE_MAX_DEV] = {};
  if (!attr_set[be_cur_dev()]) {
    hipFuncSetAttribute(reinterpret_cast<const void*>(&conv_pair_pp_kernel<NCA, INMODE, X2, RES, HEAD, STEM>),
                        hipFuncAttributeMaxDynamicSharedMemorySize, lds);
    attr_set[be_cur_dev()] = true;
  }
  if (g_pp_stamps != nullptr) {
    if (g > g_pp_stamps_cap) return -30;
    a.stamps = g_pp_stamps;
    static bool attr_st[BE_MAX_DEV] = {};
    if (!attr_st[be_cur_dev()]) {
      hipFuncSetAttribute(reinterpret_cast<const void*>(&conv_pair_pp_kernel<NCA, INMODE, X2, RES, HEAD, STEM, true>),
                          hipFuncAttributeMaxDynamicSharedMemorySize, lds);
      attr_st[be_cur_dev()] = true;
    }
    hipLaunchKernelGGL((conv_pair_pp_kernel<NCA, INMODE, X2, RES, HEAD, STEM, true>), dim3(g), dim3(ppk::NTP), lds, s, a);
    return BE_CHECK_LAUNCH();
  }
  hipLaunchKernelGGL((conv_pair_pp_kernel<NCA, INMODE, X2, RES, HEAD, STEM>), dim3(g), dim3(ppk::NTP), lds, s, a);
  return BE_CHECK_LAUNCH();
}

#include "conv_pair_pp64.inc"

template <int NCA, int INMODE, bool X2, int RES, bool PROJ = false>
int launch_pair_pp64(PairArgs a, int grid_cap, hipStream_t s) {
  constexpr int lds = PROJ ? pp64::LDS_PROJ : pp64::LDS;
  a.tiles_x = (a.W + pp64::TS - 1) / pp64::TS;
  a.tiles_y = (a.H + pp64::TS - 1) / pp64::TS;
  const int tiles = a.N * a.tiles_x * a.tiles_y;
  int g = grid_cap > 0 ? grid_cap : 256;
  if (g > tiles) g = tiles;
  if (g < 1) return 0;
  a.stamps = nullptr;
  static bool attr_set[BE_MAX_DEV] = {};
  if (!attr_set[be_cur_dev()]) {
    (void)hipFuncSetAttribute(reinterpret_cast<const void*>(&pp64::conv_pair_pp64_kernel<NCA, INMODE, X2, RES, false, PROJ>),
                              hipFuncAttributeMaxDynamicSharedMemorySize, lds);
    (void)hipFuncSetAttribute(reinterpret_cast<const void*>(&pp64::conv_pair_pp64_kernel<NCA, INMODE, X2, RES, true, PROJ>),
                              hipFuncAttributeMaxDynamicSharedMemorySize, lds);
    attr_set[be_cur_dev()] = true;
  }
  if (g_pp_stamps != nullptr) {
    if (g > g_pp_stamps_cap) return -30;
    a.stamps = g_pp_stamps;
    hipLaunchKernelGGL((pp64::conv_pair_pp64_kernel<NCA, INMODE, X2, RES, true, PROJ>), dim3(g), dim3(pp64::NTP), lds, s, a);
    return BE_CHECK_LAUNCH();
  }
  hipLaunchKernelGGL((pp64::conv_pair_pp64_kernel<NCA, INMODE, X2, RES, false, PROJ>), dim3(g), dim3(pp64::NTP), lds, s, a);
  return BE_CHECK_LAUNCH();
}
}

static int g_pair_grid = be_env_int("BE_PAIR_GRID", 0);

static int g_pair_pp = be_env_int("BE_PAIR_PP", 1);

static int g_pair_pp_stem = be_env_int("BE_PAIR_PP_STEM", 1);

static bool pp_ok(const PairArgs& a, int grid_cap) {
  if (!g_pair_pp || g_pair_stamps != nullptr) return false;
  const long long tiles = (long long)a.N * ((a.W + TW - 1) / TW) * ((a.H + TH - 1) / TH);
  const int g = grid_cap > 0 ? grid_cap : 256;
  return tiles >= 2LL * g;
}

static int g_pair_pp64 = be_env_int("BE_PAIR_PP64", 1);

static bool pp64_size_ok(int N, int H, int W, int grid_cap) {
  if (!g_pair_pp64 || g_pair_stamps != nullptr) return false;
  const long long tiles = (long long)N * ((W + pp64::TS - 1) / pp64::TS) * ((H + pp64::TS - 1) / pp64::TS);
  const int g = grid_cap > 0 ? grid_cap : 256;
  return tiles >= 2LL * g;
}

static bool pp64_ok(const PairArgs& a, int grid_cap) { return a.waf && a.wbf && pp64_size_ok(a.N, a.H, a.W, grid_cap); }

static int g_pair_pp64_proj = be_env_int("BE_PAIR_PP64_PROJ", 1);

extern "C" {

int be_conv_pair_pp64_takes(int N, int H, int W) { return pp64_size_ok(N, H, W, g_pair_grid) ? 1 : 0; }

int be_conv_pair_proj_takes(int N, int H, int W) { return g_pair_pp64_proj && be_conv_pair_pp64_takes(N, H, W); }

int be_conv_pair_set_proj_fusion(int on) {
  g_pair_pp64_proj = on;
  return 0;
}

int be_conv_pair_set_grid(int blocks) {
  g_pair_grid = blocks;
  return 0;
}

int be_conv_pair_set_stamps(void* buf, int cap_workgroups) {
  g_pair_stamps = static_cast<unsigned long long*>(buf);
  g_pair_stamps_cap = buf ? cap_workgroups : 0;
  return 0;
}

int be_conv_pair_pp_set_stamps(void* buf, int cap_workgroups) {
  g_pp_stamps = static_cast<unsigned long long*>(buf);
  g_pp_stamps_cap = buf ? cap_workgroups : 0;
  return 0;
}

int be_conv_pair_lds(int cin, int cm, int inmode, int x2, int proj, int res) {
  (void)inmode; (void)x2; (void)res;
  if (cm == 32 && cin == 8 && proj) return (int)PC<8, 32, 0, false, true, 0, 1>::LDS;
  if (cm == 32 && cin == 32) return (int)PC<32, 32, 0, false, false, 1, 1>::LDS;
  if (cm == 32 && cin == 64) return (int)PC<32, 32, 1, true, false, 2, 2>::LDS;
  if (cm == 64) return (int)PC<32, 64, 0, false, false, 1, 2>::LDS;
  return -1;
}

int be_conv_pair_frag(const void* x, const void* x2, const float* sa, const float* ta, int ta_ns, const float* sb,
                      const float* tb, int tb_ns, const float* sp, const float* tp, const void* wa, const void* wb,
                      const void* wp, const float* bias, const void* res, void* out, int N, int H, int W, int Hs,
                      int Ws, int Cin, int CM, int inmode, int proj, int resmode, const void* waf, const void* wbf,
                      hipStream_t stream) {
  PairArgs a;
  a.waf = (const bf16_t*)waf; a.wbf = (const bf16_t*)wbf; a.wpf = nullptr; a.biasp = nullptr;
  a.x = (const bf16_t*)x; a.x2 = (const bf16_t*)x2;
  a.sa = sa; a.ta = ta; a.ta_ns = ta_ns; a.sb = sb; a.tb = tb; a.tb_ns = tb_ns; a.sp = sp; a.tp = tp;
  a.wa = (const bf16_t*)wa; a.wb = (const bf16_t*)wb; a.wp = (const bf16_t*)wp; a.bias = bias;
  a.res = (const bf16_t*)res; a.out = (bf16_t*)out;
  a.N = N; a.H = H; a.W = W; a.Hs = Hs; a.Ws = Ws; a.Cin = Cin;
  a.sh = a.th = a.bh = nullptr; a.wh = nullptr; a.hout = nullptr; a.nh = 0;
  const bool hx2 = x2 != nullptr;
  if (!sa || !ta || !sb || !tb || !wa || !wb || !bias || !out || !x) return -20;
  if ((resmode != 0) != (res != nullptr)) return -21;
  if (proj && (!sp || !tp || !wp)) return -22;
  const int g = g_pair_grid;
  if (CM == 32 && Cin == 8 && inmode == 0 && !hx2 && proj && resmode == 0) {
    if (g_pair_pp_stem && pp_ok(a, g) && Hs == H && Ws == W)
      return launch_pair_pp<1, 0, false, 0, false, true>(a, g, stream);
    return launch_pair<8, 32, 0, false, true, 0, 1>(a, g, stream);
  }
  if (CM == 32 && Cin == 32 && inmode == 0 && !hx2 && !proj && resmode == 1) {
    if (pp_ok(a, g) && Hs == H && Ws == W) return launch_pair_pp<1, 0, false, 1, false>(a, g, stream);
    return launch_pair<32, 32, 0, false, false, 1, 1>(a, g, stream);
  }
  if (CM == 32 && Cin == 64 && inmode == 1 && hx2 && !proj && resmode == 2) {
    if (pp_ok(a, g) && 2 * Hs == H && 2 * Ws == W)
      return launch_pair_pp<2, 1, true, 2, false>(a, g, stream);
    return launch_pair<32, 32, 1, true, false, 2, 2>(a, g, stream);
  }
  if (CM == 64 && Cin == 32 && inmode == 2 && !hx2 && !proj && resmode == 1) {
    if (pp64_ok(a, g) && Hs == 2 * H && Ws == 2 * W) return launch_pair_pp64<1, 2, false, 1>(a, g, stream);
    return launch_pair<32, 64, 2, false, false, 1, 1>(a, g, stream);
  }
  if (CM == 64 && Cin == 64 && inmode == 0 && !hx2 && !proj && resmode == 1) {
    if (pp64_ok(a, g) && Hs == H && Ws == W) return launch_pair_pp64<2, 0, false, 1>(a, g, stream);
    return launch_pair<32, 64, 0, false, false, 1, 2>(a, g, stream);
  }
  if (CM == 64 && Cin == 128 && inmode == 1 && hx2 && !proj && resmode == 2) {
    if (pp64_ok(a, g) && 2 * Hs == H && 2 * Ws == W) return launch_pair_pp64<4, 1, true, 2>(a, g, stream);
    return launch_pair<32, 64, 1, true, false, 2, 4>(a, g, stream);
  }
  return -23;
}

int be_conv_pair_proj(const void* x, const float* sa, const float* ta, int ta_ns, const float* sb, const float* tb,
                      int tb_ns, const float* sp, const float* tp, const void* wa, const void* wb, const float* bias,
                      const float* biasp, void* out, int N, int H, int W, int Hs, int Ws, int Cin, int CM,
                      const void* waf, const void* wbf, const void* wpf, hipStream_t stream) {
  if (!x || !sa || !ta || !sb || !tb || !wa || !wb || !bias || !out) return -20;
  if (!sp || !tp || !wpf || !biasp || !waf || !wbf) return -22;
  if (CM != 64 || Cin != 32 || Hs != 2 * H || Ws != 2 * W) return -23;
  if (!be_conv_pair_proj_takes(N, H, W)) return -25;
  PairArgs a;
  a.waf = (const bf16_t*)waf; a.wbf = (const bf16_t*)wbf; a.wpf = (const bf16_t*)wpf; a.biasp = biasp;
  a.x = (const bf16_t*)x; a.x2 = nullptr;
  a.sa = sa; a.ta = ta; a.ta_ns = ta_ns; a.sb = sb; a.tb = tb; a.tb_ns = tb_ns; a.sp = sp; a.tp = tp;
  a.wa = (const bf16_t*)wa; a.wb = (const bf16_t*)wb; a.wp = nullptr; a.bias = bias;
  a.res = nullptr; a.out = (bf16_t*)out;
  a.N = N; a.H = H; a.W = W; a.Hs = Hs; a.Ws = Ws; a.Cin = Cin;
  a.sh = a.th = a.bh = nullptr; a.wh = nullptr; a.hout = nullptr; a.nh = 0;
  return launch_pair_pp64<1, 2, false, 0, true>(a, g_pair_grid, stream);
}

int be_conv_pair(const void* x, const void* x2, const float* sa, const float* ta, int ta_ns, const float* sb,
                 const float* tb, int tb_ns, const float* sp, const float* tp, const void* wa, const void* wb,
                 const void* wp, const float* bias, const void* res, void* out, int N, int H, int W, int Hs, int Ws,
                 int Cin, int CM, int inmode, int proj, int resmode, hipStream_t stream) {
  return be_conv_pair_frag(x, x2, sa, ta, ta_ns, sb, tb, tb_ns, sp, tp, wa, wb, wp, bias, res, out, N, H, W, Hs, Ws, Cin,
                           CM, inmode, proj, resmode, nullptr, nullptr, stream);
}

int be_conv_pair_head(const void* x, const float* sa, const float* ta, int ta_ns, const float* sb, const float* tb,
                      int tb_ns, const void* wa, const void* wb, const float* bias, const void* res, const float* sh,
                      const float* th, const void* wh, const float* bh, float* hout, int nh, int N, int H, int W,
                      hipStream_t stream) {
  if (!x || !sa || !ta || !sb || !tb || !wa || !wb || !bias || !res || !sh || !th || !wh || !bh || !hout) return -20;
  if (nh < 1 || nh > 16) return -24;
  PairArgs a;
  a.x = (const bf16_t*)x; a.x2 = nullptr;
  a.sa = sa; a.ta = ta; a.ta_ns = ta_ns; a.sb = sb; a.tb = tb; a.tb_ns = tb_ns; a.sp = nullptr; a.tp = nullptr;
  a.wa = (const bf16_t*)wa; a.wb = (const bf16_t*)wb; a.wp = nullptr; a.bias = bias;
  a.res = (const bf16_t*)res; a.out = nullptr; a.waf = a.wbf = nullptr; a.wpf = nullptr; a.biasp = nullptr;
  a.sh = sh; a.th = th; a.wh = (const bf16_t*)wh; a.bh = bh; a.hout = hout; a.nh = nh;
  a.N = N; a.H = H; a.W = W; a.Hs = H; a.Ws = W; a.Cin = 32;
  if (pp_ok(a, g_pair_grid)) return launch_pair_pp<1, 0, false, 1, true>(a, g_pair_grid, stream);
  return launch_pair<32, 32, 0, false, false, 1, 1, true>(a, g_pair_grid, stream);
}

}
```

csrc/kernels/conv_pp128.hip:

```cpp
#include "common.h"

namespace {
namespace pp128 {
constexpr int TH = 8, TW = 28;
constexpr int GW = 4, GT = GW * 64, NTP = 2 * GT;
constexpr int IH = TH + 2, IW = TW + 2, IPIX = IH * IW;
constexpr int IN_B = IPIX * 64;
constexpr int LDS = 2 * IN_B;
constexpr int NF = 14, FC = 7;
constexpr int NCH = 4;
constexpr int C = 128;
constexpr int HU = IPIX * 4, HUPT = (HU + GT - 1) / GT;
constexpr int WD = 3;
constexpr int WSTEP = 8 * 64 * 8;
constexpr int BD = 6, BR = 7;
static_assert(IW % 4 == 2, "the swizzle derivation needs 30 y = 2 y (mod 4)");
constexpr int PJ_B = TH * TW * 128;
constexpr int LDS_PROJ = LDS + 2 * PJ_B;
static_assert(LDS_PROJ <= 128 * 1024, "LDS budget of the ping-pong kernels");
static_assert(BD < BR, "ring");

struct Args {
  const bf16_t* x = nullptr;
  const float* sa = nullptr;
  const float* ta = nullptr;
  const bf16_t* wf = nullptr;
  const float* bias = nullptr;
  const bf16_t* res = nullptr;
  bf16_t* out = nullptr;
  int N = 0, H = 0, W = 0;
  int sa_ns = 0, ta_ns = 0;
  int relu = 0;
  int res_up2 = 0;
  int tiles_x = 0, tiles_y = 0;
  const float* sp = nullptr;
  const float* tp = nullptr;
  const bf16_t* wpf = nullptr;
  const float* bias_p = nullptr;
  bf16_t* out2 = nullptr;
  unsigned long long* stamps = nullptr;
  const float* qs = nullptr;
  const float* qt = nullptr;
  int qrelu = 0;
};

struct TileXY {
  int n, ty0, tx0;
};

__device__ __forceinline__ TileXY tile_of(const Args& a, int t) {
  const int tpi = a.tiles_x * a.tiles_y;
  TileXY r;
  r.n = t / tpi;
  const int q = t - r.n * tpi;
  r.ty0 = (q / a.tiles_x) * TH;
  r.tx0 = (q % a.tiles_x) * TW;
  return r;
}

template <bool POOL>
struct Halo {
  u32x4 h[HUPT];
  float4 aff[4];
};

template <>
struct Halo<true> {
  u32x4 h[HUPT], hb[HUPT];
  u32x4 q[HUPT], qb[HUPT];
  float4 aff[4];
  float4 affp[4];
};

template <bool POOL>
__device__ __forceinline__ void issue_aff(const Args& a, TileXY t, int c, Halo<POOL>& hr) {
  hr.aff[0] = hr.aff[1] = make_float4(1.f, 1.f, 1.f, 1.f);
  hr.aff[2] = hr.aff[3] = make_float4(0.f, 0.f, 0.f, 0.f);
  if (a.sa) {
    const float* sr = a.sa + (size_t)t.n * a.sa_ns + c;
    hr.aff[0] = *reinterpret_cast<const float4*>(sr);
    hr.aff[1] = *reinterpret_cast<const float4*>(sr + 4);
  }
  if (a.ta) {
    const float* tr = a.ta + (size_t)t.n * a.ta_ns + c;
    hr.aff[2] = *reinterpret_cast<const float4*>(tr);
    hr.aff[3] = *reinterpret_cast<const float4*>(tr + 4);
  }
}

__device__ __forceinline__ size_t pool_src(const Args& a, int n, int gy, int gx, int row, int c) {
  return (((size_t)n * 2 * a.H + 2 * gy + row) * 2 * a.W + 2 * gx) * 64 + c;
}

template <bool POOL>
__device__ __forceinline__ void issue_halo(const Args& a, TileXY t, int ch, int gt, Halo<POOL>& hr) {
  const int c = ch * 32 + (gt & 3) * 8;
  if constexpr (!POOL) issue_aff(a, t, c, hr);
#pragma unroll
  for (int i = 0; i < HUPT; ++i) {
    const int pi = min(gt + i * GT, HU - 1) >> 2;
    const int y = pi / IW, x = pi - y * IW;
    const int gy = min(max(t.ty0 - 1 + y, 0), a.H - 1);
    const int gx = min(max(t.tx0 - 1 + x, 0), a.W - 1);
    if constexpr (POOL) {
      const bf16_t* p = a.x + pool_src(a, t.n, gy, gx, 0, c);
      hr.h[i] = *reinterpret_cast<const u32x4*>(p);
      hr.hb[i] = *reinterpret_cast<const u32x4*>(p + 64);
    } else {
      hr.h[i] = *reinterpret_cast<const u32x4*>(a.x + (((size_t)t.n * a.H + gy) * a.W + gx) * C + c);
    }
  }
}

__device__ __forceinline__ void issue_halo_b(const Args& a, TileXY t, int ch, int gt, Halo<true>& hr) {
  const int c = ch * 32 + (gt & 3) * 8;
  issue_aff(a, t, c, hr);
#pragma unroll
  for (int i = 0; i < HUPT; ++i) {
    const int pi = min(gt + i * GT, HU - 1) >> 2;
    const int y = pi / IW, x = pi - y * IW;
    const int gy = min(max(t.ty0 - 1 + y, 0), a.H - 1);
    const int gx = min(max(t.tx0 - 1 + x, 0), a.W - 1);
    const bf16_t* p = a.x + pool_src(a, t.n, gy, gx, 1, c);
    hr.q[i] = *reinterpret_cast<const u32x4*>(p);
    hr.qb[i] = *reinterpret_cast<const u32x4*>(p + 64);
  }
}

__device__ __forceinline__ void issue_affp(const Args& a, int ch, int gt, Halo<true>& hr) {
  const int c = ch * 32 + (gt & 3) * 8;
  hr.affp[0] = *reinterpret_cast<const float4*>(a.sp + c);
  hr.affp[1] = *reinterpret_cast<const float4*>(a.sp + c + 4);
  hr.affp[2] = *reinterpret_cast<const float4*>(a.tp + c);
  hr.affp[3] = *reinterpret_cast<const float4*>(a.tp + c + 4);
}

__device__ __forceinline__ uint32_t max_bf16x2(uint32_t p, uint32_t q) {
  const float lo = fmaxf(lo_bf(p), lo_bf(q)), hi = fmaxf(hi_bf(p), hi_bf(q));
  return (__float_as_uint(lo) >> 16) | (__float_as_uint(hi) & 0xffff0000u);
}

__device__ __forceinline__ void reduce_a(Halo<true>& hr) {
#pragma unroll
  for (int i = 0; i < HUPT; ++i)
#pragma unroll
    for (int j = 0; j < 4; ++j) hr.h[i][j] = max_bf16x2(hr.h[i][j], hr.hb[i][j]);
}

__device__ __forceinline__ void reduce_b(Halo<true>& hr) {
#pragma unroll
  for (int i = 0; i < HUPT; ++i)
#pragma unroll
    for (int j = 0; j < 4; ++j) hr.h[i][j] = max_bf16x2(hr.h[i][j], max_bf16x2(hr.q[i][j], hr.qb[i][j]));
}

template <bool POOL>
__device__ __forceinline__ void commit(const Args& a, TileXY t, int gt, const Halo<POOL>& hr, unsigned char* rin) {
  const int c = gt & 3;
  const float sc[8] = {hr.aff[0].x, hr.aff[0].y, hr.aff[0].z, hr.aff[0].w, hr.aff[1].x, hr.aff[1].y, hr.aff[1].z, hr.aff[1].w};
  const float sh[8] = {hr.aff[2].x, hr.aff[2].y, hr.aff[2].z, hr.aff[2].w, hr.aff[3].x, hr.aff[3].y, hr.aff[3].z, hr.aff[3].w};
  const bool relu = a.relu != 0;
#pragma unroll
  for (int i = 0; i < HUPT; ++i) {
    const int u = gt + i * GT;
    if (u >= HU) continue;
    const int pi = u >> 2;
    const int y = pi / IW, x = pi - y * IW;
    const int gy = t.ty0 - 1 + y, gx = t.tx0 - 1 + x;
    u32x4 pk = (u32x4){0u, 0u, 0u, 0u};
    if (gy >= 0 && gy < a.H && gx >= 0 && gx < a.W) {
#pragma unroll
      for (int j = 0; j < 4; ++j) {
        const float lo = lo_bf(hr.h[i][j]), hi = hi_bf(hr.h[i][j]);
        pk[j] = pack2bf(fmaf(lo, sc[2 * j], sh[2 * j]), fmaf(hi, sc[2 * j + 1], sh[2 * j + 1]));
        if (relu) pk[j] = relu_bf16x2(pk[j]);
      }
    }
    *reinterpret_cast<u32x4*>(rin + pi * 64 + ((c ^ (((x >> 1) & 1) << 1)) << 4)) = pk;
  }
}

__device__ __forceinline__ void commit_proj(int ch, int gt, const Halo<true>& hr, unsigned char* rpj) {
  const int c = gt & 3;
  const float sc[8] = {hr.affp[0].x, hr.affp[0].y, hr.affp[0].z, hr.affp[0].w, hr.affp[1].x, hr.affp[1].y, hr.affp[1].z, hr.affp[1].w};
  const float sh[8] = {hr.affp[2].x, hr.affp[2].y, hr.affp[2].z, hr.affp[2].w, hr.affp[3].x, hr.affp[3].y, hr.affp[3].z, hr.affp[3].w};
#pragma unroll
  for (int i = 0; i < HUPT; ++i) {
    const int u = gt + i * GT;
    if (u >= HU) continue;
    const int pi = u >> 2;
    const int y = pi / IW, x = pi - y * IW;
    if (y < 1 || y > TH || x < 1 || x > TW) continue;
    const int py = y - 1, px = x - 1;
    u32x4 pj;
#pragma unroll
    for (int j = 0; j < 4; ++j)
      pj[j] = pack2bf(fmaf(lo_bf(hr.h[i][j]), sc[2 * j], sh[2 * j]), fmaf(hi_bf(hr.h[i][j]), sc[2 * j + 1], sh[2 * j + 1]));
    *reinterpret_cast<u32x4*>(rpj + (py * TW + px) * 128 + (((ch * 4 + c) ^ (((px >> 1) & 1) << 1) ^ ((py & 1) << 2)) << 4)) = pj;
  }
}

struct WPre {
  bf16x8 w[WD][2];
};

__device__ __forceinline__ const bf16_t* w_lane(const bf16_t* wf, int cp, int lane) {
  return wf + cp * 2 * 512 + lane * 8;
}

__device__ __forceinline__ void issue_w(const bf16_t* wl, WPre& p) {
#pragma unroll
  for (int d = 0; d < WD; ++d)
#pragma unroll
    for (int ct = 0; ct < 2; ++ct) p.w[d][ct] = *reinterpret_cast<const bf16x8*>(wl + d * WSTEP + ct * 512);
}

__device__ __forceinline__ void mma_chunk(f32x4 (&acc)[2][NF], const unsigned char* rin, const bf16_t* wl, const WPre& pre,
                                          const int (&A0)[3]) {
  bf16x8 w[9][2];
#pragma unroll
  for (int d = 0; d < WD; ++d) {
    w[d][0] = pre.w[d][0];
    w[d][1] = pre.w[d][1];
  }
  auto rd = [&](int f) {
    const int s = f / NF, j = f % NF, dy = s / 3, dx = s % 3;
    return *reinterpret_cast<const bf16x8*>(rin + A0[dx] + ((4 * (j / FC) + dy) * IW + 4 * (j % FC)) * 64);
  };
  bf16x8 bf[BR];
#pragma unroll
  for (int f = 0; f < BD; ++f) bf[f] = rd(f);
#pragma unroll
  for (int s = 0; s < 9; ++s) {
    if (s + WD < 9) {
#pragma unroll
      for (int ct = 0; ct < 2; ++ct)
        w[s + WD][ct] = *reinterpret_cast<const bf16x8*>(wl + (s + WD) * WSTEP + ct * 512);
    }
    __builtin_amdgcn_sched_barrier(0);
#pragma unroll
    for (int j = 0; j < NF; ++j) {
      const int f = s * NF + j;
      if (f + BD < 9 * NF) bf[(f + BD) % BR] = rd(f + BD);
#pragma unroll
      for (int ct = 0; ct < 2; ++ct)
        acc[ct][j] = __builtin_amdgcn_mfma_f32_16x16x32_bf16(w[s][ct], bf[f % BR], acc[ct][j], 0, 0, 0);
      __builtin_amdgcn_sched_barrier(0);
    }
  }
}

__device__ __forceinline__ void proj_mma(f32x4 (&acc)[2][NF], const unsigned char* rpj, const bf16_t* wl, int lrow, int kq) {
  bf16x8 w[2][2];
#pragma unroll
  for (int s = 0; s < 2; ++s)
#pragma unroll
    for (int ct = 0; ct < 2; ++ct) w[s][ct] = *reinterpret_cast<const bf16x8*>(wl + s * WSTEP + ct * 512);
  const int ly = lrow >> 2, lx = lrow & 3;
  const int P0 = (ly * TW + lx) * 128 + ((kq ^ (((lx >> 1) & 1) << 1) ^ ((ly & 1) << 2)) << 4);
#pragma unroll
  for (int i = 0; i < 2; ++i)
#pragma unroll
    for (int j = 0; j < NF; ++j) acc[i][j] = (f32x4){0.f, 0.f, 0.f, 0.f};
  auto rd = [&](int f) {
    const int s = f / NF, j = f % NF;
    return *reinterpret_cast<const bf16x8*>(rpj + (P0 ^ (s << 6)) + (4 * (j / FC) * TW + 4 * (j % FC)) * 128);
  };
  constexpr int PD = 3, PR = 4;
  bf16x8 bf[PR];
#pragma unroll
  for (int f = 0; f < PD; ++f) bf[f] = rd(f);
  __builtin_amdgcn_sched_barrier(0);
#pragma unroll
  for (int f = 0; f < 2 * NF; ++f) {
    if (f + PD < 2 * NF) bf[(f + PD) % PR] = rd(f + PD);
#pragma unroll
    for (int ct = 0; ct < 2; ++ct)
      acc[ct][f % NF] = __builtin_amdgcn_mfma_f32_16x16x32_bf16(w[f / NF][ct], bf[f % PR], acc[ct][f % NF], 0, 0, 0);
    __builtin_amdgcn_sched_barrier(0);
  }
}

template <int RES, bool FULL>
__device__ __forceinline__ void epilogue(const Args& a, TileXY t, const f32x4 (&acc)[2][NF], int cp, int lrow, int kq,
                                         bool act) {
  const int ly = lrow >> 2, lx = lrow & 3;
  const int co = cp * 32 + kq * 4;
  const int img_b = a.H * a.W * C * 2;
  const size_t img = (size_t)t.n * a.H * a.W * C;
  const int Wr = a.W >> 1;
  const __amdgpu_buffer_rsrc_t rr = __builtin_amdgcn_make_buffer_rsrc(
      const_cast<bf16_t*>(RES == 2 ? a.res + (size_t)t.n * (a.H >> 1) * Wr * C : (RES ? a.res + img : a.x)), (short)0,
      RES == 2 ? (a.H >> 1) * Wr * C * 2 : (RES ? img_b : 0), 0x00020000);
  const __amdgpu_buffer_rsrc_t ro = __builtin_amdgcn_make_buffer_rsrc(a.out + img, (short)0, img_b, 0x00020000);
  const __amdgpu_buffer_rsrc_t rb = __builtin_amdgcn_make_buffer_rsrc(
      const_cast<float*>(a.bias ? a.bias : a.sa), (short)0, a.bias ? C * 4 : 0, 0x00020000);
  auto voff = [&](int j, int y, int x) {
    if constexpr (FULL) return (((t.ty0 + y) * a.W + t.tx0 + x) * C + co) * 2;
    const int py = t.ty0 + 4 * (j / FC) + y, px = t.tx0 + 4 * (j % FC) + x;
    return (py < a.H && px < a.W) ? ((py * a.W + px) * C + co) * 2 : 0x7ffffff0;
  };
  auto soff = [&](int j) { return FULL ? ((j / FC) * 4 * a.W + (j % FC) * 4) * C * 2 : 0; };
  auto voff_r = [&](int j, int y, int x) {
    if constexpr (FULL) return ((((t.ty0 + y) >> 1) * Wr + ((t.tx0 + x) >> 1)) * C + co) * 2;
    const int py = t.ty0 + 4 * (j / FC) + y, px = t.tx0 + 4 * (j % FC) + x;
    return (py < a.H && px < a.W) ? (((py >> 1) * Wr + (px >> 1)) * C + co) * 2 : 0x7ffffff0;
  };
  auto soff_r = [&](int j) { return FULL ? ((j / FC) * 2 * Wr + (j % FC) * 2) * C * 2 : 0; };
  u32x2 rv[RES ? NF : 1][2];
  f32x4 bias[2];
#pragma unroll
  for (int ct = 0; ct < 2; ++ct)
    bias[ct] = __builtin_bit_cast(f32x4, __builtin_amdgcn_raw_buffer_load_b128(rb, (co + ct * 16) * 4, 0, 0));
  if constexpr (RES != 0) {
#pragma unroll
    for (int j = 0; j < NF; ++j) {
      const int o = RES == 2 ? voff_r(j, ly, lx) : voff(j, ly, lx);
      const int so = RES == 2 ? soff_r(j) : soff(j);
#pragma unroll
      for (int ct = 0; ct < 2; ++ct) rv[j][ct] = __builtin_amdgcn_raw_buffer_load_b64(rr, o + ct * 32, so, 0);
    }
  } else {
#pragma unroll
    for (int ct = 0; ct < 2; ++ct) bias[ct] = bias[ct] + (f32x4){0.f, 0.f, 0.f, 0.f};
  }
  __builtin_amdgcn_sched_barrier(0);
  int sy = ly, sx = lx;
  asm volatile("" : "+v"(sy), "+v"(sx));
#pragma unroll
  for (int j = 0; j < NF; ++j) {
    const int o = act ? voff(j, sy, sx) : 0x7ffffff0;
#pragma unroll
    for (int ct = 0; ct < 2; ++ct) {
      u32x2 st;
      if constexpr (RES != 0) {
        const u32x2 r = rv[j][ct];
        st[0] = pack2bf(acc[ct][j][0] + bias[ct][0] + lo_bf(r[0]), acc[ct][j][1] + bias[ct][1] + hi_bf(r[0]));
        st[1] = pack2bf(acc[ct][j][2] + bias[ct][2] + lo_bf(r[1]), acc[ct][j][3] + bias[ct][3] + hi_bf(r[1]));
      } else {
        st[0] = pack2bf(acc[ct][j][0] + bias[ct][0], acc[ct][j][1] + bias[ct][1]);
        st[1] = pack2bf(acc[ct][j][2] + bias[ct][2], acc[ct][j][3] + bias[ct][3]);
      }
      __builtin_amdgcn_raw_buffer_store_b64(st, ro, o + ct * 32, soff(j), 0);
    }
  }
}

template <bool FULL>
__device__ __forceinline__ void epilogue_c256(const Args& a, TileXY t, int half, const f32x4 (&acc)[2][NF], int cp, int lrow,
                                              int kq, bool act) {
  constexpr int CO = 2 * C;
  const int ly = lrow >> 2, lx = lrow & 3;
  const int co = half * C + cp * 32 + kq * 4;
  const int img_b = a.H * a.W * CO * 2;
  const __amdgpu_buffer_rsrc_t ro =
      __builtin_amdgcn_make_buffer_rsrc(a.out + (size_t)t.n * a.H * a.W * CO, (short)0, img_b, 0x00020000);
  const __amdgpu_buffer_rsrc_t rb = __builtin_amdgcn_make_buffer_rsrc(
      const_cast<float*>(a.bias ? a.bias : a.qs), (short)0, a.bias ? CO * 4 : 0, 0x00020000);
  const __amdgpu_buffer_rsrc_t rs = __builtin_amdgcn_make_buffer_rsrc(const_cast<float*>(a.qs), (short)0, CO * 4, 0x00020000);
  const __amdgpu_buffer_rsrc_t rt = __builtin_amdgcn_make_buffer_rsrc(const_cast<float*>(a.qt), (short)0, CO * 4, 0x00020000);
  auto voff = [&](int j, int y, int x) {
    if constexpr (FULL) return (((t.ty0 + y) * a.W + t.tx0 + x) * CO + co) * 2;
    const int py = t.ty0 + 4 * (j / FC) + y, px = t.tx0 + 4 * (j % FC) + x;
    return (py < a.H && px < a.W) ? ((py * a.W + px) * CO + co) * 2 : 0x7ffffff0;
  };
  auto soff = [&](int j) { return FULL ? ((j / FC) * 4 * a.W + (j % FC) * 4) * CO * 2 : 0; };
  f32x4 bias[2], qs[2], qt[2];
#pragma unroll
  for (int ct = 0; ct < 2; ++ct) {
    bias[ct] = __builtin_bit_cast(f32x4, __builtin_amdgcn_raw_buffer_load_b128(rb, (co + ct * 16) * 4, 0, 0));
    qs[ct] = __builtin_bit_cast(f32x4, __builtin_amdgcn_raw_buffer_load_b128(rs, (co + ct * 16) * 4, 0, 0));
    qt[ct] = __builtin_bit_cast(f32x4, __builtin_amdgcn_raw_buffer_load_b128(rt, (co + ct * 16) * 4, 0, 0));
    bias[ct] = bias[ct] + (f32x4){0.f, 0.f, 0.f, 0.f};
  }
  const bool qrelu = a.qrelu != 0;
  __builtin_amdgcn_sched_barrier(0);
#pragma unroll
  for (int j = 0; j < NF; ++j) {
    const int o = act ? voff(j, ly, lx) : 0x7ffffff0;
#pragma unroll
    for (int ct = 0; ct < 2; ++ct) {
      const uint32_t p0 = pack2bf(acc[ct][j][0] + bias[ct][0], acc[ct][j][1] + bias[ct][1]);
      const uint32_t p1 = pack2bf(acc[ct][j][2] + bias[ct][2], acc[ct][j][3] + bias[ct][3]);
      u32x2 st;
      st[0] = pack2bf(fmaf(lo_bf(p0), qs[ct][0], qt[ct][0]), fmaf(hi_bf(p0), qs[ct][1], qt[ct][1]));
      st[1] = pack2bf(fmaf(lo_bf(p1), qs[ct][2], qt[ct][2]), fmaf(hi_bf(p1), qs[ct][3], qt[ct][3]));
      if (qrelu) {
        st[0] = relu_bf16x2(st[0]);
        st[1] = relu_bf16x2(st[1]);
      }
      __builtin_amdgcn_raw_buffer_store_b64(st, ro, o + ct * 32, soff(j), 0);
    }
  }
}

template <bool STAMP = false, bool POOL = false, bool PROJ = false, bool C256 = false>
__global__ __launch_bounds__(NTP, 2) void conv_pp128_kernel(Args a) {
  static_assert(POOL || !PROJ, "the projection reads the pooled input");
  static_assert(!(POOL && C256), "the 256-channel build reads a plain 128-channel input");
  constexpr int NC = POOL ? 2 : NCH;
  unsigned long long ph_work[5] = {0, 0, 0, 0, 0}, ph_wait[5] = {0, 0, 0, 0, 0};
  unsigned long long tstamp = STAMP ? __builtin_amdgcn_s_memtime() : 0;
  auto pre = [&](int i) {
    if constexpr (STAMP) {
      const unsigned long long tn = __builtin_amdgcn_s_memtime();
      ph_work[i] += tn - tstamp;
      tstamp = tn;
    }
  };
  auto post = [&](int i) {
    if constexpr (STAMP) {
      const unsigned long long tn = __builtin_amdgcn_s_memtime();
      ph_wait[i] += tn - tstamp;
      tstamp = tn;
    }
  };
  auto slot = [](int c) { return c > 0 ? 2 : 0; };
  extern __shared__ __attribute__((aligned(16))) unsigned char smem[];
  const int tid0 = threadIdx.x;
  const int total = a.N * a.tiles_x * a.tiles_y * (C256 ? 2 : 1);
  auto tile_at = [&](int item) { return tile_of(a, C256 ? item >> 1 : item); };
  const int t0 = (int)(((long long)blockIdx.x * total) / gridDim.x);
  const int t1 = (int)(((long long)(blockIdx.x + 1) * total) / gridDim.x);
  if (t0 >= t1) return;
  const int grp = __builtin_amdgcn_readfirstlane(tid0 / GT);
  const int gt0 = tid0 & (GT - 1);
  unsigned char* reg = smem + grp * IN_B;
  unsigned char* rpj = PROJ ? smem + LDS + grp * PJ_B : nullptr;
  Halo<POOL> halo;
  issue_halo(a, tile_at(min(t0 + grp, t1 - 1)), 0, gt0, halo);
  if constexpr (POOL) issue_halo_b(a, tile_at(min(t0 + grp, t1 - 1)), 0, gt0, halo);
  if constexpr (PROJ) issue_affp(a, 0, gt0, halo);
  if (grp == 1) __builtin_amdgcn_s_barrier();
  const int iters = (t1 - t0 + 1) >> 1;
  for (int k = 0; k < iters; ++k) {
    int gt = gt0;
    asm volatile("" : "+v"(gt));
    const int cp = __builtin_amdgcn_readfirstlane(gt >> 6), lane = gt & 63, lrow = lane & 15, kq = lane >> 4;
    const int t = t0 + 2 * k + grp;
    const bool act = t < t1;
    const TileXY cur = tile_at(act ? t : t1 - 1);
    const bf16_t* wl = w_lane(C256 ? a.wf + ((act ? t : t1 - 1) & 1) * (NCH * 9 * WSTEP) : a.wf, cp, lane);
    int A0[3];
#pragma unroll
    for (int dx = 0; dx < 3; ++dx) {
      const int x = (lrow & 3) + dx;
      A0[dx] = ((lrow >> 2) * IW + x) * 64 + ((kq ^ (((x >> 1) & 1) << 1)) << 4);
    }
    f32x4 acc[2][NF];
#pragma unroll
    for (int i = 0; i < 2; ++i)
#pragma unroll
      for (int j = 0; j < NF; ++j) acc[i][j] = (f32x4){0.f, 0.f, 0.f, 0.f};
    WPre wpre;
#pragma unroll
    for (int c = 0; c < NC; ++c) {
      int gc = gt0;
      asm volatile("" : "+v"(gc));
      if constexpr (POOL) {
        reduce_a(halo);
        if (c > 0) {
          __builtin_amdgcn_sched_barrier(0);
          issue_halo_b(a, cur, c, gc, halo);
        }
        reduce_b(halo);
        if constexpr (PROJ) {
          if (c > 0) {
            __builtin_amdgcn_sched_barrier(0);
            issue_affp(a, c, gc, halo);
          }
        }
      }
      commit(a, cur, gc, halo, reg);
      if constexpr (PROJ) {
        __builtin_amdgcn_sched_barrier(0);
        commit_proj(c, gc, halo, rpj);
      }
      __builtin_amdgcn_sched_barrier(0);
      if (c + 1 < NC)
        issue_halo(a, cur, c + 1, gc, halo);
      else
        issue_halo(a, tile_at(min(t + 2, t1 - 1)), 0, gc, halo);
      issue_w(wl + c * 9 * WSTEP, wpre);
      pre(slot(c));
      __syncthreads();
      post(slot(c));
      __builtin_amdgcn_s_setprio(1);
      mma_chunk(acc, reg, wl + c * 9 * WSTEP, wpre, A0);
      __builtin_amdgcn_s_setprio(0);
      pre(slot(c) + 1);
      __syncthreads();
      post(slot(c) + 1);
    }
    int g3 = gt0;
    asm volatile("" : "+v"(g3));
    const bool full = cur.ty0 + TH <= a.H && cur.tx0 + TW <= a.W;
    if constexpr (POOL) {
      if constexpr (!PROJ) {
        issue_halo_b(a, tile_at(min(t + 2, t1 - 1)), 0, g3, halo);
        __builtin_amdgcn_sched_barrier(0);
      }
      if (full)
        epilogue<0, true>(a, cur, acc, cp, g3 & 15, (g3 & 63) >> 4, act);
      else
        epilogue<0, false>(a, cur, acc, cp, g3 & 15, (g3 & 63) >> 4, act);
      if constexpr (PROJ) {
        __builtin_amdgcn_sched_barrier(0);
        int g4 = gt0;
        asm volatile("" : "+v"(g4));
        proj_mma(acc, rpj, w_lane(a.wpf, cp, g4 & 63), g4 & 15, (g4 & 63) >> 4);
        Args b = a;
        b.out = a.out2;
        b.bias = a.bias_p;
        if (full)
          epilogue<0, true>(b, cur, acc, cp, g4 & 15, (g4 & 63) >> 4, act);
        else
          epilogue<0, false>(b, cur, acc, cp, g4 & 15, (g4 & 63) >> 4, act);
        __builtin_amdgcn_sched_barrier(0);
        issue_halo_b(a, tile_at(min(t + 2, t1 - 1)), 0, g4, halo);
        issue_affp(a, 0, g4, halo);
      }
    } else if constexpr (C256) {
      const int half = (act ? t : t1 - 1) & 1;
      if (full)
        epilogue_c256<true>(a, cur, half, acc, cp, g3 & 15, (g3 & 63) >> 4, act);
      else
        epilogue_c256<false>(a, cur, half, acc, cp, g3 & 15, (g3 & 63) >> 4, act);
    } else if (a.res != nullptr && a.res_up2) {
      if (full)
        epilogue<2, true>(a, cur, acc, cp, g3 & 15, (g3 & 63) >> 4, act);
      else
        epilogue<2, false>(a, cur, acc, cp, g3 & 15, (g3 & 63) >> 4, act);
    } else if (a.res != nullptr) {
      if (full)
        epilogue<1, true>(a, cur, acc, cp, g3 & 15, (g3 & 63) >> 4, act);
      else
        epilogue<1, false>(a, cur, acc, cp, g3 & 15, (g3 & 63) >> 4, act);
    } else {
      if (full)
        epilogue<0, true>(a, cur, acc, cp, g3 & 15, (g3 & 63) >> 4, act);
      else
        epilogue<0, false>(a, cur, acc, cp, g3 & 15, (g3 & 63) >> 4, act);
    }
    pre(4);
    __syncthreads();
    post(4);
  }
  if (grp == 0) __builtin_amdgcn_s_barrier();
  if constexpr (STAMP) {
    if ((tid0 & (GT - 1)) < 16) {
      const int k = tid0 & 15;
      unsigned long long v = 0;
#pragma unroll
      for (int i = 0; i < 5; ++i) {
        if (k == i) v = ph_work[i];
        if (k == 8 + i) v = ph_wait[i];
      }
      if (k == 15) v = (unsigned long long)iters;
      a.stamps[((size_t)blockIdx.x * 2 + grp) * 16 + k] = v;
    }
  }
}
}

int g_pp128 = be_env_int("BE_CONV_PP128", 1);

int g_pp128_res_up2 = be_env_int("BE_CONV_PP128_RES_UP2", 1);

int g_pp128_pool = be_env_int("BE_CONV_PP128_POOL", 1);

int g_pp128_pool_proj = be_env_int("BE_CONV_PP128_POOL_PROJ", 1);

int g_l3_prepool = be_env_int("BE_CPNET_L3_PREPOOL", 1);

int g_pp128_c256 = be_env_int("BE_CONV_PP128_C256", 1);

int g_pp128_c256_launches = 0;
int g_pp128_grid = 0;
int g_pp128_launches = 0;
int g_pp128_pool_launches = 0;
unsigned long long* g_pp128_stamps = nullptr;
int g_pp128_stamps_cap = 0;

int pp128_grid_for(int N, int H, int W, int* tiles_x, int* tiles_y, int halves = 1) {
  if (!g_pp128 || N <= 0 || H <= 0 || W <= 0 || (long long)H * W * 256 * halves >= (1LL << 31) - 64) return 0;
  const int tx = (W + pp128::TW - 1) / pp128::TW, ty = (H + pp128::TH - 1) / pp128::TH;
  const long long tiles = (long long)N * tx * ty * halves;
  const bool forced = g_pp128_grid > 0;
  const int g = forced ? (int)(tiles < g_pp128_grid ? tiles : g_pp128_grid) : 256;
  if (!(forced || tiles >= 2LL * g) || tiles >= (1LL << 30)) return 0;
  if (tiles_x) *tiles_x = tx;
  if (tiles_y) *tiles_y = ty;
  return g;
}

pp128::Args pp128_args(const void* x, const float* pscale, const float* pshift, int pshift_ns, int pscale_ns, int prelu,
                       const void* wfrag, const float* bias, void* out, int N, int H, int W) {
  pp128::Args a;
  a.x = (const bf16_t*)x; a.sa = pscale; a.ta = pshift; a.sa_ns = pscale_ns; a.ta_ns = pshift_ns;
  a.wf = (const bf16_t*)wfrag; a.bias = bias; a.out = (bf16_t*)out;
  a.N = N; a.H = H; a.W = W; a.relu = prelu & 1;
  a.stamps = g_pp128_stamps;
  return a;
}

template <bool POOL, bool PROJ, bool C256>
int pp128_launch(const pp128::Args& a, int grid, hipStream_t stream) {
  constexpr int lds = PROJ ? pp128::LDS_PROJ : pp128::LDS;
  if constexpr (PROJ) {
    static bool attr_set[BE_MAX_DEV] = {};
    if (!attr_set[be_cur_dev()]) {
      if (hipFuncSetAttribute(reinterpret_cast<const void*>(&pp128::conv_pp128_kernel<false, POOL, PROJ, C256>),
                              hipFuncAttributeMaxDynamicSharedMemorySize, lds) != hipSuccess ||
          hipFuncSetAttribute(reinterpret_cast<const void*>(&pp128::conv_pp128_kernel<true, POOL, PROJ, C256>),
                              hipFuncAttributeMaxDynamicSharedMemorySize, lds) != hipSuccess)
        return -33;
      attr_set[be_cur_dev()] = true;
    }
  }
  if (a.stamps != nullptr) {
    if (grid > g_pp128_stamps_cap) return -30;
    hipLaunchKernelGGL((pp128::conv_pp128_kernel<true, POOL, PROJ, C256>), dim3(grid), dim3(pp128::NTP), lds, stream, a);
  } else {
    hipLaunchKernelGGL((pp128::conv_pp128_kernel<false, POOL, PROJ, C256>), dim3(grid), dim3(pp128::NTP), lds, stream, a);
  }
  return BE_CHECK_LAUNCH();
}

}

extern "C" {

int be_conv2d_nhwc(const void* x, const void* x2, const float* pscale, const float* pshift, int pshift_ns, int pscale_ns,
                   int prelu, const void* w, const float* bias, const void* res, void* out, int N, int H, int W,
                   int Hs, int Ws, int Cin, int Cout, int cout_valid, int ks, int ck, int tco, int inmode,
                   int out_f32_nchw, int nw, const float* qscale, const float* qshift, int qshift_ns,
                   hipStream_t stream);

int be_conv_pp128_set_grid(int blocks) {
  g_pp128_grid = blocks;
  return 0;
}

int be_conv_pp128_set_stamps(void* buf, int cap_workgroups) {
  g_pp128_stamps = static_cast<unsigned long long*>(buf);
  g_pp128_stamps_cap = buf ? cap_workgroups : 0;
  return 0;
}

int be_conv_pp128_launches() { return g_pp128_launches; }

int be_conv2d_nhwc_frag_res(const void* x, const void* x2, const float* pscale, const float* pshift, int pshift_ns,
                            int pscale_ns, int prelu, const void* w, const float* bias, const void* res, void* out,
                            int N, int H, int W, int Hs, int Ws, int Cin, int Cout, int cout_valid, int ks, int ck,
                            int tco, int inmode, int out_f32_nchw, int nw, const float* qscale, const float* qshift,
                            int qshift_ns, const void* wfrag, int res_up2, hipStream_t stream) {
  const bool frag_ok = wfrag && ks == 3 && ck == 32 && !x2 && !out_f32_nchw && Cout == 128 && !(prelu & 2) && !qscale &&
                       !qshift && x && out;
  const bool shape_ok = frag_ok && inmode == 0 && Cin == 128 && Hs == H && Ws == W;
  if (res_up2 && !(shape_ok && res && H % 2 == 0 && W % 2 == 0)) return -31;
  const bool pool_ok = frag_ok && g_pp128_pool && inmode == 2 && Cin == 64 && Hs == 2 * H && Ws == 2 * W && !res;
  if (shape_ok || pool_ok) {
    pp128::Args a = pp128_args(x, pscale, pshift, pshift_ns, pscale_ns, prelu, wfrag, bias, out, N, H, W);
    const int g = pp128_grid_for(N, H, W, &a.tiles_x, &a.tiles_y);
    if (g > 0 && pool_ok) {
      ++g_pp128_pool_launches;
      return pp128_launch<true, false, false>(a, g, stream);
    }
    if (g > 0) {
      a.res = (const bf16_t*)res;
      a.res_up2 = res_up2 ? 1 : 0;
      ++g_pp128_launches;
      return pp128_launch<false, false, false>(a, g, stream);
    }
  }
  if (res_up2) return -31;
  return be_conv2d_nhwc(x, x2, pscale, pshift, pshift_ns, pscale_ns, prelu, w, bias, res, out, N, H, W, Hs, Ws, Cin, Cout,
                        cout_valid, ks, ck, tco, inmode, out_f32_nchw, nw, qscale, qshift, qshift_ns, stream);
}

int be_conv2d_nhwc_frag(const void* x, const void* x2, const float* pscale, const float* pshift, int pshift_ns,
                        int pscale_ns, int prelu, const void* w, const float* bias, const void* res, void* out, int N,
                        int H, int W, int Hs, int Ws, int Cin, int Cout, int cout_valid, int ks, int ck, int tco,
                        int inmode, int out_f32_nchw, int nw, const float* qscale, const float* qshift, int qshift_ns,
                        const void* wfrag, hipStream_t stream) {
  return be_conv2d_nhwc_frag_res(x, x2, pscale, pshift, pshift_ns, pscale_ns, prelu, w, bias, res, out, N, H, W, Hs, Ws,
                                 Cin, Cout, cout_valid, ks, ck, tco, inmode, out_f32_nchw, nw, qscale, qshift,
                                 qshift_ns, wfrag, 0, stream);
}

int be_conv_pp128_takes(int N, int H, int W) { return pp128_grid_for(N, H, W, nullptr, nullptr) > 0 ? 1 : 0; }

int be_conv_pp128_takes_pool(int N, int Hs, int Ws) {
  return g_pp128_pool && Hs % 2 == 0 && Ws % 2 == 0 && pp128_grid_for(N, Hs / 2, Ws / 2, nullptr, nullptr) > 0 ? 1 : 0;
}

int be_conv_pp128_set_pool(int pool, int pool_proj) {
  g_pp128_pool = pool;
  g_pp128_pool_proj = pool_proj;
  return 0;
}

int be_conv_pp128_pool_launches() { return g_pp128_pool_launches; }

int be_conv_pp128_takes_pool_proj(int N, int Hs, int Ws) {
  return g_pp128_pool_proj && be_conv_pp128_takes_pool(N, Hs, Ws);
}

int be_conv_pp128_pool_proj(const void* x, const float* pscale, const float* pshift, int pshift_ns, int pscale_ns, int prelu,
                            const void* wfrag, const float* bias, void* out, const float* sp, const float* tp,
                            const void* wpfrag, const float* bias_p, void* out2, int N, int Hs, int Ws,
                            hipStream_t stream) {
  if (!x || !wfrag || !out || !sp || !tp || !wpfrag || !out2 || out == out2 || (prelu & ~1)) return -32;
  if (!be_conv_pp128_takes_pool_proj(N, Hs, Ws)) return -32;
  pp128::Args a = pp128_args(x, pscale, pshift, pshift_ns, pscale_ns, prelu, wfrag, bias, out, N, Hs / 2, Ws / 2);
  const int g = pp128_grid_for(N, Hs / 2, Ws / 2, &a.tiles_x, &a.tiles_y);
  a.sp = sp; a.tp = tp; a.wpf = (const bf16_t*)wpfrag; a.bias_p = bias_p; a.out2 = (bf16_t*)out2;
  ++g_pp128_pool_launches;
  return pp128_launch<true, true, false>(a, g, stream);
}

static int pp128_c256_grid_for(int N, int H, int W, int* tiles_x, int* tiles_y) {
  return pp128_grid_for(N, H, W, tiles_x, tiles_y, 2);
}

int be_conv_pp128_takes_prepool(int N, int H, int W) {
  return g_l3_prepool && pp128_c256_grid_for(N, H, W, nullptr, nullptr) > 0 ? 1 : 0;
}

int be_conv_pp128_takes_c256(int N, int H, int W) { return g_pp128_c256 && be_conv_pp128_takes_prepool(N, H, W); }

int be_conv_pp128_set_c256(int prepool, int c256) {
  g_l3_prepool = prepool;
  g_pp128_c256 = c256;
  return 0;
}

int be_conv_pp128_c256_launches() { return g_pp128_c256_launches; }

int be_conv_pp128_c256(const void* x, const float* pscale, const float* pshift, int pshift_ns, int pscale_ns, int prelu,
                       const void* wfrag, const float* bias, void* out, const float* qscale, const float* qshift, int N,
                       int H, int W, hipStream_t stream) {
  if (!x || !wfrag || !out || x == out || !qscale || !qshift || (prelu & ~3)) return -34;
  if (!be_conv_pp128_takes_c256(N, H, W)) return -34;
  pp128::Args a = pp128_args(x, pscale, pshift, pshift_ns, pscale_ns, prelu, wfrag, bias, out, N, H, W);
  const int g = pp128_c256_grid_for(N, H, W, &a.tiles_x, &a.tiles_y);
  a.qs = qscale; a.qt = qshift; a.qrelu = (prelu >> 1) & 1;
  ++g_pp128_c256_launches;
  return pp128_launch<false, false, true>(a, g, stream);
}

int be_conv_pp128_takes_res_up2(int N, int H, int W) {
  return g_pp128_res_up2 && H % 2 == 0 && W % 2 == 0 && be_conv_pp128_takes(N, H, W);
}

}
```

Before: 2591 img/s.

## Permute output-channel weight rows so epilogues issue contiguous 128-bit stores

```diff
diff --git a/bioengine_worker_amd/models/cpnet.py b/bioengine_worker_amd/models/cpnet.py
--- a/bioengine_worker_amd/models/cpnet.py
+++ b/bioengine_worker_amd/models/cpnet.py
@@ -194,6 +194,7 @@
         self.pc = convops.PackedConv.from_weight(conv.weight, conv.bias, cin_pad=cin_pad, cout_pad_to=cout_pad_to).to(device)
         if convops.pp128_build(self.pc) is not None and torch.device(device).type == "cuda":
             self.pc.frag()
+            self.pc.frag8()
         s, t = _bn_fold(bn, device)
         self.scale = _pad_vec(s, self.pc.cin_pad, 0.0)
         self.shift = _pad_vec(t, self.pc.cin_pad, 0.0)
diff --git a/bioengine_worker_amd/ops/conv.py b/bioengine_worker_amd/ops/conv.py
--- a/bioengine_worker_amd/ops/conv.py
+++ b/bioengine_worker_amd/ops/conv.py
@@ -34,6 +34,8 @@
     wp: torch.Tensor | None = None
     wf: torch.Tensor | None = None
     wf_key: tuple | None = None
+    wf8: torch.Tensor | None = None
+    wf8_key: tuple | None = None
 
     @staticmethod
     def choose(cin_pad: int, cout: int, ks: int = 3) -> tuple[int, int]:
@@ -85,11 +87,15 @@
         if self.bias is not None:
             self.bias = self.bias.to(device)
         built = self.wp is not None and self.frag_built() is not None
+        built8 = self.wp is not None and self.frag8_built() is not None
         if self.wp is not None:
             self.wp = self.wp.to(device)
         if built:
             self.wf = self.wf.to(device)
             self.wf_key = self._wp_key()
+        if built8:
+            self.wf8 = self.wf8.to(device)
+            self.wf8_key = self._wp_key()
         return self
 
     def refresh(self, weight: torch.Tensor, bias: torch.Tensor | None = None) -> None:
@@ -98,6 +104,7 @@
             self.bias = bias.detach().float()
         self.wp = self._pack(self.w)
         self.wf = self.wf_key = None
+        self.wf8 = self.wf8_key = None
 
     def _wp_key(self) -> tuple:
         return (self.wp.data_ptr(), self.wp._version, str(self.wp.device))
@@ -113,6 +120,21 @@
         if self.wf is not None and self.wf_key == self._wp_key() and self.wf.device == self.wp.device:
             return self.wf
         return None
+
+    def frag8(self) -> torch.Tensor:
+        if self.frag8_built() is None:
+            pack = pack_frag_c256 if pp128_build(self) == "c256" else pack_frag if self.ks == 3 else pack_frag_1x1
+            self.wf8 = pack(self.wp.index_select(0, frag8_rows(self.wp.shape[0]).to(self.wp.device)))
+            self.wf8_key = self._wp_key()
+        return self.wf8
+
+    def frag8_built(self) -> torch.Tensor | None:
+        if self.wf8 is not None and self.wf8_key == self._wp_key() and self.wf8.device == self.wp.device:
+            return self.wf8
+        return None
+
+    def frag8_for_launch(self) -> torch.Tensor | None:
+        return self.frag8() if self.frag_built() is not None else None
 
 
 PP128_BUILDS = {(3, 128, 128): "c128", (3, 64, 128): "pool", (1, 64, 128): "proj", (3, 128, 256): "c256"}
@@ -179,6 +201,13 @@
 
 def pp128_takes_res_up2(pc: PackedConv, x: torch.Tensor) -> bool:
     return not x.is_cuda or _pp128_takes("res_up2", x, (pc, "c128"))
+
+
+def frag8_rows(cout: int) -> torch.Tensor:
+    assert cout % 32 == 0, "whole 32-channel pairs"
+    r = torch.arange(cout)
+    p, ct, kq, i = r // 32, (r // 16) % 2, (r // 4) % 4, r % 4
+    return 32 * p + 8 * kq + 4 * ct + i
 
 
 def pack_frag_1x1(wp: torch.Tensor) -> torch.Tensor:
@@ -354,7 +383,7 @@
     if post_scale is not None:
         assert post_scale.dtype == torch.float32 and post_scale.is_contiguous() and post_scale.numel() == pc.cout
     build = pp128_build(pc)
-    wf = pc.frag_built() if build == "c128" or (build == "pool" and inmode == "pool2") else None
+    wf = pc.frag8_for_launch() if build == "c128" or (build == "pool" and inmode == "pool2") else None
     args = (
         _native.ptr(x), _native.ptr(x2), _native.ptr(scale), _native.ptr(shift), pshift_ns, pscale_ns,
         int(bool(relu)) | (2 if post_relu else 0),
@@ -375,7 +404,7 @@
     N, Hs, Ws, Cin = x.shape
     assert x.is_cuda and x.dtype == torch.bfloat16 and x.is_contiguous() and Cin == 64 == pc.cin_pad == pp.cin_pad
     assert frag_eligible_pool(pc) and frag_eligible_proj(pp)
-    wf, wpf = pc.frag_built(), pp.frag_built()
+    wf, wpf = pc.frag8_for_launch(), pp.frag8_for_launch()
     assert wf is not None and wpf is not None, "fragment-order weights are packed when the engine is built"
     assert proj_scale.dtype == proj_shift.dtype == torch.float32 and proj_scale.numel() == proj_shift.numel() == 64
     assert proj_scale.is_contiguous() and proj_shift.is_contiguous()
@@ -419,7 +448,7 @@
     N, H, W, Cin = x.shape
     assert x.is_cuda and x.dtype == torch.bfloat16 and x.is_contiguous() and Cin == 128 == pc.cin_pad
     assert frag_eligible_c256(pc)
-    wf = pc.frag_built()
+    wf = pc.frag8_for_launch()
     assert wf is not None, "fragment-order weights are packed when the engine is built"
     for q in (post_scale, post_shift):
         assert q is not None and q.dtype == torch.float32 and q.is_contiguous() and q.dim() == 1 and q.numel() == 256
diff --git a/csrc/kernels/conv_pair.hip b/csrc/kernels/conv_pair.hip
--- a/csrc/kernels/conv_pair.hip
+++ b/csrc/kernels/conv_pair.hip
@@ -129,6 +129,8 @@
 static_assert(GW == 4 || GW == 8, "group size");
 }
 
+__device__ __forceinline__ int pp_row8(int r) { return ((r >> 2) & 3) * 8 + (r >> 4) * 4 + (r & 3); }
+
 struct PPHalo {
   u32x4 h[ppk::HUPT];
   float4 aff[4];
@@ -255,7 +257,7 @@
 }
 
 struct PPSkip {
-  u32x2 xv[ppk::APT][2];
+  u32x4 xv[ppk::APT];
 };
 
 __device__ __forceinline__ bool pp_last(int gw, int lrow, int& ry, int& rx) {
@@ -281,9 +283,7 @@
       pp_last(gw, lrow, ry, rx);
     }
     const int gy = min(max(t.ty0 - 1 + ry, 0), a.H - 1), gx = min(max(t.tx0 - 1 + rx, 0), a.W - 1);
-    const bf16_t* xp = a.x2 + (((size_t)t.n * a.H + gy) * a.W + gx) * 32 + kq * 4;
-#pragma unroll
-    for (int ct = 0; ct < 2; ++ct) sk.xv[j][ct] = *reinterpret_cast<const u32x2*>(xp + ct * 16);
+    sk.xv[j] = *reinterpret_cast<const u32x4*>(a.x2 + (((size_t)t.n * a.H + gy) * a.W + gx) * 32 + kq * 8);
   }
 }
 
@@ -291,35 +291,37 @@
 __device__ __forceinline__ void pp_epi_a(const PairArgs& a, TileXY t, const f32x4 (&acc)[2][ppk::APT],
                                          unsigned char* rh, const float4 (&s)[2], const float4 (&sh)[2],
                                          const PPSkip& sk, int gw, int lrow, int kq) {
-#pragma unroll
-  for (int ct = 0; ct < 2; ++ct) {
-    const int hc = ((2 * ct) | (kq >> 1));
-    const int hw = (((gw >> 1) * RW + (gw & 1) * 16 + lrow) * 64) + ((hc ^ ((lrow >> 1) & 3)) << 4) + (kq & 1) * 8;
-#pragma unroll
-    for (int j = 0; j < ppk::APT; ++j) {
-      int ry, rx, off;
-      if (j < ppk::APT - 1) {
-        ry = (gw >> 1) + (ppk::GW / 2) * j;
-        rx = (gw & 1) * 16 + lrow;
-        off = hw + j * (ppk::GW / 2) * RW * 64;
-      } else {
-        if (!pp_last(gw, lrow, ry, rx)) continue;
-        off = (ry * RW + rx) * 64 + ((hc ^ ((rx >> 1) & 3)) << 4) + (kq & 1) * 8;
-      }
-      const int gy = t.ty0 - 1 + ry, gx = t.tx0 - 1 + rx;
-      float v0 = acc[ct][j][0], v1 = acc[ct][j][1], v2 = acc[ct][j][2], v3 = acc[ct][j][3];
-      if constexpr (X2) {
-        u32x2 xv = sk.xv[j][ct];
-        asm volatile("" : "+v"(xv));
-        v0 += lo_bf(xv[0]); v1 += hi_bf(xv[0]); v2 += lo_bf(xv[1]); v3 += hi_bf(xv[1]);
-      }
-      u32x2 st = (u32x2){0u, 0u};
-      if (INT || (gy >= 0 && gy < a.H && gx >= 0 && gx < a.W)) {
-        st[0] = relu_bf16x2(pack2bf(fmaf(v0, s[ct].x, sh[ct].x), fmaf(v1, s[ct].y, sh[ct].y)));
-        st[1] = relu_bf16x2(pack2bf(fmaf(v2, s[ct].z, sh[ct].z), fmaf(v3, s[ct].w, sh[ct].w)));
-      }
-      *reinterpret_cast<u32x2*>(rh + off) = st;
-    }
+  const int hw = (((gw >> 1) * RW + (gw & 1) * 16 + lrow) * 64) + ((kq ^ ((lrow >> 1) & 3)) << 4);
+#pragma unroll
+  for (int j = 0; j < ppk::APT; ++j) {
+    int ry, rx, off;
+    if (j < ppk::APT - 1) {
+      ry = (gw >> 1) + (ppk::GW / 2) * j;
+      rx = (gw & 1) * 16 + lrow;
+      off = hw + j * (ppk::GW / 2) * RW * 64;
+    } else {
+      if (!pp_last(gw, lrow, ry, rx)) continue;
+      off = (ry * RW + rx) * 64 + ((kq ^ ((rx >> 1) & 3)) << 4);
+    }
+    const int gy = t.ty0 - 1 + ry, gx = t.tx0 - 1 + rx;
+    u32x4 xv = (u32x4){0u, 0u, 0u, 0u};
+    if constexpr (X2) {
+      xv = sk.xv[j];
+      asm volatile("" : "+v"(xv));
+    }
+    u32x4 st = (u32x4){0u, 0u, 0u, 0u};
+    if (INT || (gy >= 0 && gy < a.H && gx >= 0 && gx < a.W)) {
+#pragma unroll
+      for (int ct = 0; ct < 2; ++ct) {
+        float v0 = acc[ct][j][0], v1 = acc[ct][j][1], v2 = acc[ct][j][2], v3 = acc[ct][j][3];
+        if constexpr (X2) {
+          v0 += lo_bf(xv[2 * ct]); v1 += hi_bf(xv[2 * ct]); v2 += lo_bf(xv[2 * ct + 1]); v3 += hi_bf(xv[2 * ct + 1]);
+        }
+        st[2 * ct] = relu_bf16x2(pack2bf(fmaf(v0, s[ct].x, sh[ct].x), fmaf(v1, s[ct].y, sh[ct].y)));
+        st[2 * ct + 1] = relu_bf16x2(pack2bf(fmaf(v2, s[ct].z, sh[ct].z), fmaf(v3, s[ct].w, sh[ct].w)));
+      }
+    }
+    *reinterpret_cast<u32x4*>(rh + off) = st;
   }
 }
 
@@ -362,76 +364,56 @@
 }
 
 struct PPRes {
-  u32x2 rv[ppk::BPT][2];
+  u32x4 rv[ppk::BPT];
   float4 bias[2];
 };
 
-template <int RES>
+template <int RES, bool N8>
 __device__ __forceinline__ void pp_issue_res(const PairArgs& a, TileXY t, int gw, int lrow, int kq, PPRes& r) {
 #pragma unroll
   for (int pt = 0; pt < ppk::BPT; ++pt) {
     if constexpr (RES == 0) {
-      r.rv[pt][0] = r.rv[pt][1] = (u32x2){0u, 0u};
+      r.rv[pt] = (u32x4){0u, 0u, 0u, 0u};
       continue;
     }
     const int py = min(t.ty0 + ppk::RPW * gw + (pt >> 1), a.H - 1), px = min(t.tx0 + (pt & 1) * 16 + lrow, a.W - 1);
-    const bf16_t* rp = RES == 1 ? a.res + (((size_t)t.n * a.H + py) * a.W + px) * 32 + kq * 4
-                                : a.res + (((size_t)t.n * (a.H >> 1) + (py >> 1)) * (a.W >> 1) + (px >> 1)) * 32 + kq * 4;
-#pragma unroll
-    for (int ct = 0; ct < 2; ++ct) r.rv[pt][ct] = *reinterpret_cast<const u32x2*>(rp + ct * 16);
-  }
-#pragma unroll
-  for (int ct = 0; ct < 2; ++ct) r.bias[ct] = *reinterpret_cast<const float4*>(a.bias + ct * 16 + kq * 4);
+    const bf16_t* rp = RES == 1 ? a.res + (((size_t)t.n * a.H + py) * a.W + px) * 32
+                                : a.res + (((size_t)t.n * (a.H >> 1) + (py >> 1)) * (a.W >> 1) + (px >> 1)) * 32;
+    if constexpr (N8) {
+      r.rv[pt] = *reinterpret_cast<const u32x4*>(rp + kq * 8);
+    } else {
+#pragma unroll
+      for (int ct = 0; ct < 2; ++ct) {
+        const u32x2 v = *reinterpret_cast<const u32x2*>(rp + ct * 16 + kq * 4);
+        r.rv[pt][2 * ct] = v[0];
+        r.rv[pt][2 * ct + 1] = v[1];
+      }
+    }
+  }
+#pragma unroll
+  for (int ct = 0; ct < 2; ++ct)
+    r.bias[ct] = *reinterpret_cast<const float4*>(a.bias + (N8 ? kq * 8 + ct * 4 : ct * 16 + kq * 4));
 }
 
 template <int RES>
 __device__ __forceinline__ void pp_epi_b(const PairArgs& a, TileXY t, const f32x4 (&acc)[2][ppk::BPT], const PPRes& r,
-                                         unsigned char* ws, int gw, int lrow, int kq, bool act) {
+                                         int gw, int lrow, int kq, bool act) {
   const __amdgpu_buffer_rsrc_t rs = __builtin_amdgcn_make_buffer_rsrc(
       a.out + (size_t)t.n * a.H * a.W * 32, (short)0, a.H * a.W * 64, 0x00020000);
-  if constexpr (PP_VAR & 16) {
-#pragma unroll
-    for (int pt = 0; pt < ppk::BPT; ++pt) {
-      const int py = t.ty0 + ppk::RPW * gw + (pt >> 1), px = t.tx0 + (pt & 1) * 16 + lrow;
-      const bool ok = act && py < a.H && px < a.W;
-#pragma unroll
-      for (int ct = 0; ct < 2; ++ct) {
-        u32x2 rv = r.rv[pt][ct];
-        asm volatile("" : "+v"(rv));
-        u32x2 st;
-        st[0] = pack2bf(acc[ct][pt][0] + r.bias[ct].x + lo_bf(rv[0]), acc[ct][pt][1] + r.bias[ct].y + hi_bf(rv[0]));
-        st[1] = pack2bf(acc[ct][pt][2] + r.bias[ct].z + lo_bf(rv[1]), acc[ct][pt][3] + r.bias[ct].w + hi_bf(rv[1]));
-        const int off = ok ? ((py * a.W + px) * 32 + ct * 16 + kq * 4) * 2 : 0x7ffffff0;
-        __builtin_amdgcn_raw_buffer_store_b64(st, rs, off, 0, 0);
-      }
-    }
-    return;
-  }
-#pragma unroll
-  for (int ct = 0; ct < 2; ++ct) {
-    const int ow = lrow * 64 + ((((2 * ct) | (kq >> 1)) ^ ((lrow >> 1) & 3)) << 4) + (kq & 1) * 8;
-#pragma unroll
-    for (int pt = 0; pt < ppk::BPT; ++pt) {
-      u32x2 rv = r.rv[pt][ct];
-      if constexpr (RES != 0) asm volatile("" : "+v"(rv));
-      u32x2 st;
-      st[0] = pack2bf(acc[ct][pt][0] + r.bias[ct].x + lo_bf(rv[0]), acc[ct][pt][1] + r.bias[ct].y + hi_bf(rv[0]));
-      st[1] = pack2bf(acc[ct][pt][2] + r.bias[ct].z + lo_bf(rv[1]), acc[ct][pt][3] + r.bias[ct].w + hi_bf(rv[1]));
-      *reinterpret_cast<u32x2*>(ws + ow + ((pt >> 1) * 32 + (pt & 1) * 16) * 64) = st;
-    }
-  }
-  __builtin_amdgcn_fence(__ATOMIC_RELEASE, "wavefront");
-  __builtin_amdgcn_wave_barrier();
-  __builtin_amdgcn_fence(__ATOMIC_ACQUIRE, "wavefront");
-  const int lane = lrow + 16 * kq;
-  const int rd = (lane >> 2) * 64 + (((lane & 3) ^ ((lane >> 3) & 3)) << 4);
-  const int py0 = t.ty0 + ppk::RPW * gw, px0 = t.tx0 + (lane >> 2);
-#pragma unroll
-  for (int it = 0; it < 2 * ppk::RPW; ++it) {
-    const int py = py0 + (it >> 1), px = px0 + (it & 1) * 16;
-    const u32x4 v = *reinterpret_cast<const u32x4*>(ws + rd + it * 1024);
-    const int off = (act && py < a.H && px < a.W) ? ((py * a.W + px) * 32 + (lane & 3) * 8) * 2 : 0x7ffffff0;
-    __builtin_amdgcn_raw_buffer_store_b128(v, rs, off, 0, 0);
+#pragma unroll
+  for (int pt = 0; pt < ppk::BPT; ++pt) {
+    const int py = t.ty0 + ppk::RPW * gw + (pt >> 1), px = t.tx0 + (pt & 1) * 16 + lrow;
+    u32x4 rv = r.rv[pt];
+    if constexpr (RES != 0) asm volatile("" : "+v"(rv));
+    u32x4 st;
+#pragma unroll
+    for (int ct = 0; ct < 2; ++ct) {
+      st[2 * ct] = pack2bf(acc[ct][pt][0] + r.bias[ct].x + lo_bf(rv[2 * ct]), acc[ct][pt][1] + r.bias[ct].y + hi_bf(rv[2 * ct]));
+      st[2 * ct + 1] =
+          pack2bf(acc[ct][pt][2] + r.bias[ct].z + lo_bf(rv[2 * ct + 1]), acc[ct][pt][3] + r.bias[ct].w + hi_bf(rv[2 * ct + 1]));
+    }
+    const int off = (act && py < a.H && px < a.W) ? ((py * a.W + px) * 32 + kq * 8) * 2 : 0x7ffffff0;
+    __builtin_amdgcn_raw_buffer_store_b128(st, rs, off, 0, 0);
     __builtin_amdgcn_sched_barrier(0);
   }
 }
@@ -446,7 +428,7 @@
     u32x4 bw;
 #pragma unroll
     for (int ct = 0; ct < 2; ++ct) {
-      u32x2 rv = r.rv[pt][ct];
+      u32x2 rv = (u32x2){r.rv[pt][2 * ct], r.rv[pt][2 * ct + 1]};
       asm volatile("" : "+v"(rv));
       const float4 bias = r.bias[ct];
       const uint32_t o0 = pack2bf(acc[ct][pt][0] + bias.x + lo_bf(rv[0]), acc[ct][pt][1] + bias.y + hi_bf(rv[0]));
@@ -615,7 +597,8 @@
       tstamp = tn;
     }
   };
-  constexpr int NST = HEAD ? 4 * ppk::BPT : ((PP_VAR & 16) ? 2 * ppk::BPT : 2 * ppk::RPW);
+  constexpr int NST = HEAD ? 4 * ppk::BPT : ppk::BPT;
+  constexpr bool B8 = !HEAD;
   extern __shared__ __attribute__((aligned(16))) unsigned char smem[];
   const int tid0 = threadIdx.x;
   const int total = a.N * a.tiles_x * a.tiles_y;
@@ -630,15 +613,17 @@
       const int r = u / 52, q = u % 52;
       const bf16_t* src;
       bf16_t* dst;
-      if (q < 12) { src = a.wa + (size_t)r * 96 + q * 8; dst = wl + r * pps::WSTRA + q * 8; }
-      else if (q < 48) { src = a.wb + (size_t)r * 288 + (q - 12) * 8; dst = const_cast<bf16_t*>(wb) + r * ppk::WSTR + (q - 12) * 8; }
-      else { src = a.wp + (size_t)r * 32 + (q - 48) * 8; dst = const_cast<bf16_t*>(wp) + r * pps::WSTRP + (q - 48) * 8; }
+      const int c = pp_row8(r);
+      if (q < 12) { src = a.wa + (size_t)c * 96 + q * 8; dst = wl + r * pps::WSTRA + q * 8; }
+      else if (q < 48) { src = a.wb + (size_t)c * 288 + (q - 12) * 8; dst = const_cast<bf16_t*>(wb) + r * ppk::WSTR + (q - 12) * 8; }
+      else { src = a.wp + (size_t)c * 32 + (q - 48) * 8; dst = const_cast<bf16_t*>(wp) + r * pps::WSTRP + (q - 48) * 8; }
       *reinterpret_cast<u32x4*>(dst) = *reinterpret_cast<const u32x4*>(src);
     }
   } else {
     for (int u = tid0; u < (NCA + 1) * 32 * 36; u += ppk::NTP) {
       const int pnl = u / (32 * 36), q = u % (32 * 36), r = q / 36, k8 = q % 36;
-      const bf16_t* src = pnl < NCA ? a.wa + ((size_t)r * NCA + pnl) * 288 + k8 * 8 : a.wb + (size_t)r * 288 + k8 * 8;
+      const int c = (pnl < NCA || B8) ? pp_row8(r) : r;
+      const bf16_t* src = pnl < NCA ? a.wa + ((size_t)c * NCA + pnl) * 288 + k8 * 8 : a.wb + (size_t)c * 288 + k8 * 8;
       *reinterpret_cast<u32x4*>(wl + pnl * 32 * ppk::WSTR + r * ppk::WSTR + k8 * 8) = *reinterpret_cast<const u32x4*>(src);
     }
   }
@@ -699,8 +684,8 @@
       if (c == NCA - 1) {
 #pragma unroll
         for (int ct = 0; ct < 2; ++ct) {
-          sb[ct] = *reinterpret_cast<const float4*>(a.sb + ct * 16 + kq * 4);
-          tb[ct] = *reinterpret_cast<const float4*>(a.tb + (size_t)cur.n * a.tb_ns + ct * 16 + kq * 4);
+          sb[ct] = *reinterpret_cast<const float4*>(a.sb + kq * 8 + ct * 4);
+          tb[ct] = *reinterpret_cast<const float4*>(a.tb + (size_t)cur.n * a.tb_ns + kq * 8 + ct * 4);
         }
         if constexpr (X2) pp_issue_skip(a, cur, gw, lrow, kq, sk);
       }
@@ -723,7 +708,7 @@
     if (inner) pp_epi_a<X2, true>(a, cur, acc_a, reg, sb, tb, sk, gw, g3 & 15, (g3 & 63) >> 4);
     else pp_epi_a<X2, false>(a, cur, acc_a, reg, sb, tb, sk, gw, g3 & 15, (g3 & 63) >> 4);
     PPRes res;
-    if constexpr (PP_VAR & 1) pp_issue_res<RES>(a, cur, gw, g3 & 15, (g3 & 63) >> 4, res);
+    if constexpr (PP_VAR & 1) pp_issue_res<RES, B8>(a, cur, gw, g3 & 15, (g3 & 63) >> 4, res);
     if constexpr (PP_VAR & 8) issue0(tile_xy(a, min(t + 2, t1 - 1)), g3);
     pre(2 * NCA);
     __syncthreads();
@@ -732,7 +717,7 @@
     asm volatile("" : "+v"(g4));
     const int lrow4 = g4 & 15, kq4 = (g4 & 63) >> 4;
     f32x4 acc_b[2][ppk::BPT];
-    if constexpr (!(PP_VAR & 1)) pp_issue_res<RES>(a, cur, gw, lrow4, kq4, res);
+    if constexpr (!(PP_VAR & 1)) pp_issue_res<RES, B8>(a, cur, gw, lrow4, kq4, res);
 #pragma unroll
     for (int i = 0; i < 2; ++i)
 #pragma unroll
@@ -751,7 +736,7 @@
     if constexpr (!(PP_VAR & 10)) next_halo();
     __builtin_amdgcn_sched_barrier(0);
     if constexpr (HEAD) pp_epi_head(a, cur, acc_b, res, hr, gw, lrow5, kq5, act);
-    else pp_epi_b<RES>(a, cur, acc_b, res, reg + gw * ppk::OUTW_B, gw, lrow5, kq5, act);
+    else pp_epi_b<RES>(a, cur, acc_b, res, gw, lrow5, kq5, act);
     if constexpr (PP_VAR & 2) next_halo();
     pre(2 * NCA + 2);
     __syncthreads();
diff --git a/csrc/kernels/conv_pp128.hip b/csrc/kernels/conv_pp128.hip
--- a/csrc/kernels/conv_pp128.hip
+++ b/csrc/kernels/conv_pp128.hip
@@ -285,7 +285,7 @@
 __device__ __forceinline__ void epilogue(const Args& a, TileXY t, const f32x4 (&acc)[2][NF], int cp, int lrow, int kq,
                                          bool act) {
   const int ly = lrow >> 2, lx = lrow & 3;
-  const int co = cp * 32 + kq * 4;
+  const int co = cp * 32 + kq * 8;
   const int img_b = a.H * a.W * C * 2;
   const size_t img = (size_t)t.n * a.H * a.W * C;
   const int Wr = a.W >> 1;
@@ -307,18 +307,17 @@
     return (py < a.H && px < a.W) ? (((py >> 1) * Wr + (px >> 1)) * C + co) * 2 : 0x7ffffff0;
   };
   auto soff_r = [&](int j) { return FULL ? ((j / FC) * 2 * Wr + (j % FC) * 2) * C * 2 : 0; };
-  u32x2 rv[RES ? NF : 1][2];
+  u32x4 rv[RES ? NF : 1];
   f32x4 bias[2];
 #pragma unroll
   for (int ct = 0; ct < 2; ++ct)
-    bias[ct] = __builtin_bit_cast(f32x4, __builtin_amdgcn_raw_buffer_load_b128(rb, (co + ct * 16) * 4, 0, 0));
+    bias[ct] = __builtin_bit_cast(f32x4, __builtin_amdgcn_raw_buffer_load_b128(rb, (co + ct * 4) * 4, 0, 0));
   if constexpr (RES != 0) {
 #pragma unroll
     for (int j = 0; j < NF; ++j) {
       const int o = RES == 2 ? voff_r(j, ly, lx) : voff(j, ly, lx);
       const int so = RES == 2 ? soff_r(j) : soff(j);
-#pragma unroll
-      for (int ct = 0; ct < 2; ++ct) rv[j][ct] = __builtin_amdgcn_raw_buffer_load_b64(rr, o + ct * 32, so, 0);
+      rv[j] = __builtin_amdgcn_raw_buffer_load_b128(rr, o, so, 0);
     }
   } else {
 #pragma unroll
@@ -330,19 +329,19 @@
 #pragma unroll
   for (int j = 0; j < NF; ++j) {
     const int o = act ? voff(j, sy, sx) : 0x7ffffff0;
+    u32x4 st;
 #pragma unroll
     for (int ct = 0; ct < 2; ++ct) {
-      u32x2 st;
       if constexpr (RES != 0) {
-        const u32x2 r = rv[j][ct];
-        st[0] = pack2bf(acc[ct][j][0] + bias[ct][0] + lo_bf(r[0]), acc[ct][j][1] + bias[ct][1] + hi_bf(r[0]));
-        st[1] = pack2bf(acc[ct][j][2] + bias[ct][2] + lo_bf(r[1]), acc[ct][j][3] + bias[ct][3] + hi_bf(r[1]));
+        const uint32_t r0 = rv[j][2 * ct], r1 = rv[j][2 * ct + 1];
+        st[2 * ct] = pack2bf(acc[ct][j][0] + bias[ct][0] + lo_bf(r0), acc[ct][j][1] + bias[ct][1] + hi_bf(r0));
+        st[2 * ct + 1] = pack2bf(acc[ct][j][2] + bias[ct][2] + lo_bf(r1), acc[ct][j][3] + bias[ct][3] + hi_bf(r1));
       } else {
-        st[0] = pack2bf(acc[ct][j][0] + bias[ct][0], acc[ct][j][1] + bias[ct][1]);
-        st[1] = pack2bf(acc[ct][j][2] + bias[ct][2], acc[ct][j][3] + bias[ct][3]);
+        st[2 * ct] = pack2bf(acc[ct][j][0] + bias[ct][0], acc[ct][j][1] + bias[ct][1]);
+        st[2 * ct + 1] = pack2bf(acc[ct][j][2] + bias[ct][2], acc[ct][j][3] + bias[ct][3]);
       }
-      __builtin_amdgcn_raw_buffer_store_b64(st, ro, o + ct * 32, soff(j), 0);
-    }
+    }
+    __builtin_amdgcn_raw_buffer_store_b128(st, ro, (int)((unsigned)o + (unsigned)soff(j)), 0, 0);
   }
 }
 
@@ -351,7 +350,7 @@
                                               int kq, bool act) {
   constexpr int CO = 2 * C;
   const int ly = lrow >> 2, lx = lrow & 3;
-  const int co = half * C + cp * 32 + kq * 4;
+  const int co = half * C + cp * 32 + kq * 8;
   const int img_b = a.H * a.W * CO * 2;
   const __amdgpu_buffer_rsrc_t ro =
       __builtin_amdgcn_make_buffer_rsrc(a.out + (size_t)t.n * a.H * a.W * CO, (short)0, img_b, 0x00020000);
@@ -368,9 +367,9 @@
   f32x4 bias[2], qs[2], qt[2];
 #pragma unroll
   for (int ct = 0; ct < 2; ++ct) {
-    bias[ct] = __builtin_bit_cast(f32x4, __builtin_amdgcn_raw_buffer_load_b128(rb, (co + ct * 16) * 4, 0, 0));
-    qs[ct] = __builtin_bit_cast(f32x4, __builtin_amdgcn_raw_buffer_load_b128(rs, (co + ct * 16) * 4, 0, 0));
-    qt[ct] = __builtin_bit_cast(f32x4, __builtin_amdgcn_raw_buffer_load_b128(rt, (co + ct * 16) * 4, 0, 0));
+    bias[ct] = __builtin_bit_cast(f32x4, __builtin_amdgcn_raw_buffer_load_b128(rb, (co + ct * 4) * 4, 0, 0));
+    qs[ct] = __builtin_bit_cast(f32x4, __builtin_amdgcn_raw_buffer_load_b128(rs, (co + ct * 4) * 4, 0, 0));
+    qt[ct] = __builtin_bit_cast(f32x4, __builtin_amdgcn_raw_buffer_load_b128(rt, (co + ct * 4) * 4, 0, 0));
     bias[ct] = bias[ct] + (f32x4){0.f, 0.f, 0.f, 0.f};
   }
   const bool qrelu = a.qrelu != 0;
@@ -378,19 +377,19 @@
 #pragma unroll
   for (int j = 0; j < NF; ++j) {
     const int o = act ? voff(j, ly, lx) : 0x7ffffff0;
+    u32x4 st;
 #pragma unroll
     for (int ct = 0; ct < 2; ++ct) {
       const uint32_t p0 = pack2bf(acc[ct][j][0] + bias[ct][0], acc[ct][j][1] + bias[ct][1]);
       const uint32_t p1 = pack2bf(acc[ct][j][2] + bias[ct][2], acc[ct][j][3] + bias[ct][3]);
-      u32x2 st;
-      st[0] = pack2bf(fmaf(lo_bf(p0), qs[ct][0], qt[ct][0]), fmaf(hi_bf(p0), qs[ct][1], qt[ct][1]));
-      st[1] = pack2bf(fmaf(lo_bf(p1), qs[ct][2], qt[ct][2]), fmaf(hi_bf(p1), qs[ct][3], qt[ct][3]));
+      st[2 * ct] = pack2bf(fmaf(lo_bf(p0), qs[ct][0], qt[ct][0]), fmaf(hi_bf(p0), qs[ct][1], qt[ct][1]));
+      st[2 * ct + 1] = pack2bf(fmaf(lo_bf(p1), qs[ct][2], qt[ct][2]), fmaf(hi_bf(p1), qs[ct][3], qt[ct][3]));
       if (qrelu) {
-        st[0] = relu_bf16x2(st[0]);
-        st[1] = relu_bf16x2(st[1]);
+        st[2 * ct] = relu_bf16x2(st[2 * ct]);
+        st[2 * ct + 1] = relu_bf16x2(st[2 * ct + 1]);
       }
-      __builtin_amdgcn_raw_buffer_store_b64(st, ro, o + ct * 32, soff(j), 0);
-    }
+    }
+    __builtin_amdgcn_raw_buffer_store_b128(st, ro, (int)((unsigned)o + (unsigned)soff(j)), 0, 0);
   }
 }
 
```

Measured after the change: 2601 img/s (median of 6 runs). About the same (+0.4%).
